# Guilucand/PanDelos

Measured on AMD Instinct MI355X. Metric: scored gene-pairs/sec (whole node), higher is better.
Workload: dtype u32 accumulate + f32 finalize

## Files before the change

pandelos_amd/csrc/pdl_api.hip:

```cpp
#include "pdl_common.h"

#include <algorithm>
#include <cstdlib>
#include <cstring>
#include <limits>

static thread_local std::string g_create_error = "";

#define PDL_GUARD_BEGIN try {
#define PDL_GUARD_END(ctx_)                                                       \
    } catch (const pdl_error &e) {                                                \
        if (ctx_) (ctx_)->err = e.msg; else g_create_error = e.msg;               \
        return e.code;                                                            \
    } catch (const std::bad_alloc &) {                                            \
        if (ctx_) (ctx_)->err = "host allocation failed";                         \
        return PDL_ERR_DEVICE;                                                    \
    }

template <class T> static T *xalloc(size_t n) {
    T *p = static_cast<T *>(malloc((n ? n : 1) * sizeof(T)));
    if (!p) throw std::bad_alloc();
    return p;
}

// ... 434 lines not shown
        ThreadCopier &tc = t_copier;
        tc.open(c->device);
        if (z) {
            tc.fetch(out->scores, c->c_score.as<float>() + z0, (size_t) z * 4);
            tc.fetch(out->percs, c->c_perc.as<float>() + z0, (size_t) z * 4);
            tc.fetch(out->tr_percs, c->c_tr.as<float>() + z0, (size_t) z * 4);
            tc.fetch(out->row, c->c_row.as<int32_t>() + z0, (size_t) z * 4);
            tc.fetch(out->column, c->c_col.as<int32_t>() + z0, (size_t) z * 4);
        }
        if (rows) tc.fetch(out->max_genome_score, c->MS.as<float>() + (size_t) p0 * G, (size_t) rows * G * 4);
        tc.fetch(out->max_genome_score_col, c->CM.as<float>() + (size_t) lg * N, (size_t) N * 4);
    }
    for (uint32_t i = 0; i < z; i++) {
        out->first_seq_genome[i] = (int32_t) c->h_genome_of[out->row[i]];
        out->second_seq_genome[i] = (int32_t) c->h_genome_of[out->column[i]];
    }
    for (uint32_t i = 0; i < N; i++) out->scoresMaxMappings[i] = std::numeric_limits<int32_t>::max();
    for (uint32_t j = 0; j < rows; j++) out->scoresMaxMappings[c->h_genome_rows[c->h_genome_row_off[genome] + j]] = (int32_t) j;
    return PDL_OK;
    } catch (const pdl_error &e) { { std::lock_guard<std::mutex> lk(c->mu); c->err = e.msg; } pdl_free_scores(out); return e.code;
    } catch (const std::bad_alloc &) { { std::lock_guard<std::mutex> lk(c->mu); c->err = "host allocation failed"; } pdl_free_scores(out); return PDL_ERR_DEVICE; }
}

void pdl_free_edges(pdl_edges *e) {
    if (!e) return;
    free(e->src); free(e->dst); free(e->score);
    memset(e, 0, sizeof(*e));
}

int pdl_compute_edges(pdl_ctx *c, uint32_t genome, pdl_edges *out) {
    if (!c || !out) return PDL_ERR_ARGUMENT;
    memset(out, 0, sizeof(*out));
    try {
    {
        std::lock_guard<std::mutex> lk(c->mu);
        int rc = c->scored ? PDL_OK : score_all_locked(c);
        if (rc != PDL_OK) return rc;
        if (genome >= c->G) PDL_FAIL(PDL_ERR_ARGUMENT, "genome %u out of range (%u genomes)", genome, c->G);
        if (c->h_local_genome[genome] < 0) PDL_FAIL(PDL_ERR_ARGUMENT, "genome %u is not in this context's shard", genome);
        if (!c->edges_valid) {
            PDL_HIP(hipSetDevice(c->device));
            pdl_run_bbh_all(c);
        }
    }
    const int32_t lg = c->h_local_genome[genome];
    const uint64_t a1 = c->h_edge1[lg], b1 = c->h_edge1[lg + 1], a2 = c->h_edge_off[lg], b2 = c->h_edge_off[lg + 1];
    const uint64_t n1 = c->n_edges1, n2 = c->n_edges - c->n_edges1;
    const uint32_t cnt = (uint32_t) ((b1 - a1) + (b2 - a2));
    out->count = cnt;
    out->src = xalloc<int32_t>(cnt); out->dst = xalloc<int32_t>(cnt); out->score = xalloc<float>(cnt);
    const uint8_t *m = c->edge_mirror;
    const size_t k1 = (size_t) (b1 - a1), k2 = (size_t) (b2 - a2);
    if (k1) {
        memcpy(out->src, m + a1 * 4, k1 * 4); memcpy(out->dst, m + n1 * 4 + a1 * 4, k1 * 4); memcpy(out->score, m + n1 * 8 + a1 * 4, k1 * 4);
    }
    if (k2) {
        const uint8_t *m2 = m + n1 * 12;
        memcpy(out->src + k1, m2 + a2 * 4, k2 * 4); memcpy(out->dst + k1, m2 + n2 * 4 + a2 * 4, k2 * 4); memcpy(out->score + k1, m2 + n2 * 8 + a2 * 4, k2 * 4);
    }
    return PDL_OK;
    } catch (const pdl_error &e) { { std::lock_guard<std::mutex> lk(c->mu); c->err = e.msg; } pdl_free_edges(out); return e.code;
    } catch (const std::bad_alloc &) { { std::lock_guard<std::mutex> lk(c->mu); c->err = "host allocation failed"; } pdl_free_edges(out); return PDL_ERR_DEVICE; }
}

void pdl_free_families(pdl_families *f) {
    if (!f) return;
    free(f->component_of); free(f->is_node); free(f->family_off); free(f->family_genes); free(f->collides);
    memset(f, 0, sizeof(*f));
}

static void fill_families(const pdl_fam_result &r, pdl_families *out) {
    out->sequences = r.sequences; out->nodes = r.nodes; out->families = r.families; out->colliding = r.colliding; out->device_ms = r.device_ms;
    out->component_of = xalloc<uint32_t>(r.component_of.size()); out->is_node = xalloc<uint8_t>(r.is_node.size());
    out->family_off = xalloc<uint32_t>(r.family_off.size()); out->family_genes = xalloc<uint32_t>(r.family_genes.size());
    out->collides = xalloc<uint8_t>(r.collides.size());
    if (!r.component_of.empty()) memcpy(out->component_of, r.component_of.data(), r.component_of.size() * 4);
    if (!r.is_node.empty()) memcpy(out->is_node, r.is_node.data(), r.is_node.size());
    memcpy(out->family_off, r.family_off.data(), r.family_off.size() * 4);
    if (!r.family_genes.empty()) memcpy(out->family_genes, r.family_genes.data(), r.family_genes.size() * 4);
    if (!r.collides.empty()) memcpy(out->collides, r.collides.data(), r.collides.size());
}

int pdl_compute_families(pdl_ctx *c, pdl_families *out) {
    if (!c || !out) return PDL_ERR_ARGUMENT;
    memset(out, 0, sizeof(*out));
    std::lock_guard<std::mutex> lk(c->mu);
    try {
        if (!c->preprocessed) PDL_FAIL(PDL_ERR_STATE, "pdl_compute_families before pdl_preprocess");
        if (c->only_complexity) PDL_FAIL(PDL_ERR_STATE, "pdl_compute_families: the context was preprocessed with only_complexity");
        if (c->dist) PDL_FAIL(PDL_ERR_STATE, "pdl_compute_families: not available on a multi-GPU context (gather the edges: pdl_families_of_edges)");
        if (c->shard_set || !c->dict_shard.empty())
            PDL_FAIL(PDL_ERR_STATE, "pdl_compute_families: a genome shard is in force, the context does not hold every genome's edges (gather them: pdl_families_of_edges)");
        int rc = c->scored ? PDL_OK : score_all_locked(c);
        if (rc != PDL_OK) return rc;
        PDL_HIP(hipSetDevice(c->device));
        if (!c->edges_valid) pdl_run_bbh_all(c);
        if (!c->fam_valid) pdl_run_families_of_context(c);
        fill_families(c->fam, out);
        return PDL_OK;
    } catch (const pdl_error &e) { c->err = e.msg; c->fam_valid = false; pdl_free_families(out); return e.code;
    } catch (const std::bad_alloc &) { c->err = "host allocation failed"; pdl_free_families(out); return PDL_ERR_DEVICE; }
}

int pdl_families_of_edges(pdl_ctx *c, const int32_t *src, const int32_t *dst, uint64_t n_edges, const uint32_t *genome_of, uint32_t n_sequences,
                          pdl_families *out) {
    if (!c || !out) return PDL_ERR_ARGUMENT;
    memset(out, 0, sizeof(*out));
    std::lock_guard<std::mutex> lk(c->mu);
    try {
        if ((n_edges && (!src || !dst)) || (n_sequences && !genome_of)) PDL_FAIL(PDL_ERR_ARGUMENT, "pdl_families_of_edges: NULL pointer");
        if (n_edges >= 0x7fffffffull || n_sequences >= 0x7fffffffu) PDL_FAIL(PDL_ERR_UNSUPPORTED, "pdl_families_of_edges: 2^31 genes or edges and more");
        PDL_HIP(hipSetDevice(c->device));
        pdl_ctx::FamBufs &b = c->fb;
        uint32_t g_max = 0;
        for (uint32_t i = 0; i < n_sequences; i++) g_max = std::max(g_max, genome_of[i]);
        if (n_edges) {
            b.up_src.alloc(n_edges * 4); b.up_dst.alloc(n_edges * 4);
            PDL_HIP(hipMemcpyAsync(b.up_src.p, src, n_edges * 4, hipMemcpyHostToDevice, c->stream));
            PDL_HIP(hipMemcpyAsync(b.up_dst.p, dst, n_edges * 4, hipMemcpyHostToDevice, c->stream));
        }
        if (n_sequences) {
            b.up_gen.alloc((size_t) n_sequences * 4);
            PDL_HIP(hipMemcpyAsync(b.up_gen.p, genome_of, (size_t) n_sequences * 4, hipMemcpyHostToDevice, c->stream));
        }
        const int32_t *s2[2] = {b.up_src.as<int32_t>(), nullptr}, *d2[2] = {b.up_dst.as<int32_t>(), nullptr};
        const uint64_t n2[2] = {n_edges, 0};
        pdl_fam_result r;
        pdl_run_families(c, s2, d2, n2, false, true, true, b.up_gen.as<uint32_t>(), n_sequences, bit_length64(g_max), r);
        fill_families(r, out);
        return PDL_OK;
    } catch (const pdl_error &e) { c->err = e.msg; pdl_free_families(out); return e.code;
    } catch (const std::bad_alloc &) { c->err = "host allocation failed"; pdl_free_families(out); return PDL_ERR_DEVICE; }
}

int pdl_set_option(pdl_ctx *c, const char *name, int64_t value) {
    if (!c || !name) return PDL_ERR_ARGUMENT;
    std::lock_guard<std::mutex> lk(c->mu);
    const std::string n(name);
    if (n == "join_tier1") {
        if (!(value == -1 || value == 0 || (value >= 9 && value <= 11) || value == 20 || value == 21)) { c->err = "join_tier1: -1, 0, 9, 10, 11, 20 or 21"; return PDL_ERR_ARGUMENT; }
        c->opt_tier1 = (int) value;
    } else if (n == "join_tier0") c->opt_tier0 = value < 0 ? -1 : (value != 0);
    else if (n == "sift_threshold") {
        if (value != 0 && value != 1) { c->err = "sift_threshold: 0 or 1"; return PDL_ERR_ARGUMENT; }
        c->opt_sift_threshold = (int) value;
    }
    else if (n == "join_tiny_tier2") c->opt_tiny_tier2 = value != 0;
    else if (n == "join_grid_pct") c->opt_grid_pct = (int) value;
    else if (n == "stage_timers") c->opt_stage_timers = value != 0;
    else if (n == "host_mirror") c->opt_host_mirror = value != 0;
    else if (n == "staging_cap") c->opt_staging_cap = value > 0 ? (uint64_t) value : 0;
    else if (n == "aside_test_reload") c->opt_aside_test_reload = value != 0;
    else if (n == "onepass_scan") c->opt_onepass_scan = value != 0;
    else if (n == "low_memory") c->opt_low_memory = value != 0;
    else if (n == "query_batch_bytes") {
        if (value <= 0) { c->err = "query_batch_bytes: a positive byte count"; return PDL_ERR_ARGUMENT; }
        c->opt_query_batch_bytes = (uint64_t) value;
        return PDL_OK;
    }
    else { c->err = "unknown option " + n; return PDL_ERR_ARGUMENT; }
    c->scored = false;
    return PDL_OK;
}

int pdl_dist_preprocess_begin(pdl_ctx *c, const uint8_t *d_residues, const uint64_t *d_offsets, const uint32_t *d_genome_of,
                              uint32_t n, uint64_t n_res, int k, uint32_t world, uint32_t rank, pdl_dist_slice *out) {
    if (!c || !out) return PDL_ERR_ARGUMENT;
    std::lock_guard<std::mutex> lk(c->mu);
    PDL_GUARD_BEGIN
    if (!d_offsets || !d_genome_of || (!d_residues && n_res)) PDL_FAIL(PDL_ERR_ARGUMENT, "null input pointer");
    if (((uintptr_t) d_residues & 15) != 0) PDL_FAIL(PDL_ERR_ARGUMENT, "d_residues must be 16-byte aligned");
    if (world == 0 || rank >= world || world > 64) PDL_FAIL(PDL_ERR_ARGUMENT, "rank %u of %u (at most 64 ranks)", rank, world);
    PDL_HIP(hipSetDevice(c->device));
    c->preprocessed = false; c->scored = false; c->tasks_ready = false; c->mirror_valid = false;
    c->dist = false; c->dist_stage = 0;
    adopt_device_input(c, d_residues, d_offsets, d_genome_of, n, n_res);
    c->N = n; c->R = n_res;
    c->U = c->Ushared = c->NG = c->P = c->M = 0;
    if (k <= 0) PDL_FAIL(PDL_ERR_KVALUE, "K value must be greater than 0.");
    if (n == 0) PDL_FAIL(PDL_ERR_EMPTY, "empty dataset");
    build_genome_layout(c);
    c->world = world; c->rank = rank;
    c->shard.clear(); c->shard_set = false; c->dict_shard.clear();
    pdl_run_dist_begin(c, k);
    out->d_postings = c->post.p; out->records = c->U_slice; out->kmers = c->M_slice;
    out->genome_weights = c->h_run_weights.data(); out->genomes = c->G;
    out->genome_costs = c->h_run_costs.data();
    return PDL_OK;
    PDL_GUARD_END(c)
}

int pdl_dist_preprocess_finish(pdl_ctx *c, void *d_postings_all, uint64_t total_records, const uint64_t *genome_weights, pdl_cost *out_cost) {
    if (!c) return PDL_ERR_ARGUMENT;
    std::lock_guard<std::mutex> lk(c->mu);
    PDL_GUARD_BEGIN
    if (!c->dist || c->dist_stage != 1) PDL_FAIL(PDL_ERR_STATE, "pdl_dist_preprocess_finish without pdl_dist_preprocess_begin");
    if (c->dist_sender) PDL_FAIL(PDL_ERR_STATE, "pdl_dist_preprocess_ranges built this run's range tuples (and took its group-head bits out): finish with pdl_dist_preprocess_finish_ranges");
    if (!d_postings_all || ((uintptr_t) d_postings_all & 7) != 0) PDL_FAIL(PDL_ERR_ARGUMENT, "the gathered dictionary must be an 8-byte aligned device array");
    if (total_records < c->U_slice) PDL_FAIL(PDL_ERR_ARGUMENT, "the gathered dictionary (%llu records) is smaller than this rank's run (%llu)",
                                             (unsigned long long) total_records, (unsigned long long) c->U_slice);
    PDL_HIP(hipSetDevice(c->device));
    c->post_ext = static_cast<uint2 *>(d_postings_all);
    pdl_run_dist_finish(c, total_records, genome_weights);
    c->preprocessed = true;
    fill_cost(c, out_cost);
    return PDL_OK;
    PDL_GUARD_END(c)
}

int pdl_dist_preprocess_ranges(pdl_ctx *c, const uint64_t *run_records, const uint64_t *genome_weights, const uint64_t *genome_costs, pdl_dist_ranges *out) {
    if (!c || !out || !run_records || !genome_weights || !genome_costs) return PDL_ERR_ARGUMENT;
    std::lock_guard<std::mutex> lk(c->mu);
    PDL_GUARD_BEGIN
    if (!c->dist || c->dist_stage != 1) PDL_FAIL(PDL_ERR_STATE, "pdl_dist_preprocess_ranges without pdl_dist_preprocess_begin");
    PDL_HIP(hipSetDevice(c->device));
    memset(out, 0, sizeof(*out));
    out->available = pdl_run_dist_ranges(c, run_records, genome_weights, genome_costs) ? 1 : 0;
    out->d_keys = c->dist_out_keys; out->d_ranges = reinterpret_cast<const uint64_t *>(c->dist_out_ranges);
    out->counts = c->h_tuple_counts.data(); out->total = c->dist_out_total;
    out->shared_records = c->dist_run_counters[0]; out->groups = c->dist_run_counters[1]; out->repeat_sample = c->dist_run_counters[2];
    return PDL_OK;
    PDL_GUARD_END(c)
}

int pdl_dist_preprocess_finish_ranges(pdl_ctx *c, void *d_postings_all, uint64_t total_records, uint32_t *d_keys, uint64_t *d_ranges, uint64_t n_tuples,
                                      const uint64_t *counter_sums, pdl_cost *out_cost) {
    if (!c || !counter_sums || ((!d_keys || !d_ranges) && n_tuples)) return PDL_ERR_ARGUMENT;
    std::lock_guard<std::mutex> lk(c->mu);
    PDL_GUARD_BEGIN
    if (!c->dist || c->dist_stage != 1 || !c->dist_sender) PDL_FAIL(PDL_ERR_STATE, "pdl_dist_preprocess_finish_ranges without a pdl_dist_preprocess_ranges that said \"available\"");
    if (!d_postings_all || ((uintptr_t) d_postings_all & 7) != 0) PDL_FAIL(PDL_ERR_ARGUMENT, "the gathered dictionary must be an 8-byte aligned device array");
    if (n_tuples && ((((uintptr_t) d_keys) & 3) != 0 || (((uintptr_t) d_ranges) & 7) != 0)) PDL_FAIL(PDL_ERR_ARGUMENT, "the received tuples must be aligned device arrays");
    PDL_HIP(hipSetDevice(c->device));
    c->post_ext = static_cast<uint2 *>(d_postings_all);
    pdl_run_dist_finish_ranges(c, total_records, d_keys, reinterpret_cast<unsigned long long *>(d_ranges), n_tuples, counter_sums);
    c->preprocessed = true;
    fill_cost(c, out_cost);
    return PDL_OK;
    PDL_GUARD_END(c)
}

int pdl_dist_genome_owner(const pdl_ctx *c, uint32_t *out) {
    if (!c || !out) return PDL_ERR_ARGUMENT;
    if (!c->dist || c->dist_stage < 2) return PDL_ERR_STATE;
    memcpy(out, c->h_owner.data(), (size_t) c->G * 4);
    return PDL_OK;
}

int pdl_dist_score_begin(pdl_ctx *c, pdl_dist_outbox *out) {
    if (!c || !out) return PDL_ERR_ARGUMENT;
    std::lock_guard<std::mutex> lk(c->mu);
    PDL_GUARD_BEGIN
    if (!c->dist || c->dist_stage < 2) PDL_FAIL(PDL_ERR_STATE, "pdl_dist_score_begin before pdl_dist_preprocess_finish");
    PDL_HIP(hipSetDevice(c->device));
    c->scored = false; c->mirror_valid = false; c->edges_valid = false; c->dist_stage = 2;
    pdl_run_dist_score_begin(c);
    out->d_cells = c->outbox.as<pdl_dist_cell>();
    out->counts = c->h_outbox_counts.data();
    out->total = 0;
    for (uint64_t v : c->h_outbox_counts) out->total += v;
    return PDL_OK;
    PDL_GUARD_END(c)
}

int pdl_dist_score_finish(pdl_ctx *c, const pdl_dist_cell *d_inbox, uint64_t n_inbox) {
    if (!c || (!d_inbox && n_inbox)) return PDL_ERR_ARGUMENT;
    std::lock_guard<std::mutex> lk(c->mu);
    PDL_GUARD_BEGIN
    if (!c->dist || c->dist_stage != 3) PDL_FAIL(PDL_ERR_STATE, "pdl_dist_score_finish without pdl_dist_score_begin");
    if (n_inbox >= 0xffffffffull) PDL_FAIL(PDL_ERR_UNSUPPORTED, "more than 2^32 received cells");
    PDL_HIP(hipSetDevice(c->device));
    pdl_run_dist_score_finish(c, d_inbox, n_inbox);
    return PDL_OK;
    PDL_GUARD_END(c)
}

int pdl_copy_device(pdl_ctx *c, void *d_dst, const void *d_src, uint64_t bytes) {
    if (!c || ((!d_dst || !d_src) && bytes)) return PDL_ERR_ARGUMENT;
    std::lock_guard<std::mutex> lk(c->mu);
    PDL_GUARD_BEGIN
    PDL_HIP(hipSetDevice(c->device));
    if (bytes) PDL_HIP(hipMemcpyAsync(d_dst, d_src, bytes, hipMemcpyDeviceToDevice, c->stream));
    PDL_HIP(hipStreamSynchronize(c->stream));
    return PDL_OK;
    PDL_GUARD_END(c)
}

int pdl_get_dictionary(pdl_ctx *c, uint64_t *ranks, uint32_t *seqs, uint32_t *counts) {
    if (!c) return PDL_ERR_ARGUMENT;
    std::lock_guard<std::mutex> lk(c->mu);
    PDL_GUARD_BEGIN
    if (!c->preprocessed) PDL_FAIL(PDL_ERR_STATE, "pdl_get_dictionary before pdl_preprocess");
    if (c->dist) PDL_FAIL(PDL_ERR_STATE, "pdl_get_dictionary: a multi-GPU context keeps ranks only for its own interval");
    if (!c->keys_b.p || !c->recpos.p) PDL_FAIL(PDL_ERR_STATE, "pdl_get_dictionary: the sorted k-mer stream was released (option low_memory)");
    PDL_HIP(hipSetDevice(c->device));
    const uint64_t U = c->U, M = c->M;
    std::vector<uint32_t> recpos(U);
    std::vector<uint2> post(U);
    PDL_HIP(hipMemcpyAsync(recpos.data(), c->recpos.p, U * 4, hipMemcpyDeviceToHost, c->stream));
    PDL_HIP(hipMemcpyAsync(post.data(), c->post.p, U * 8, hipMemcpyDeviceToHost, c->stream));
    std::vector<uint8_t> keys(M * (c->key64 ? 8 : 4));
    PDL_HIP(hipMemcpyAsync(keys.data(), c->keys_b.p, keys.size(), hipMemcpyDeviceToHost, c->stream));
    PDL_HIP(hipStreamSynchronize(c->stream));
    for (uint64_t u = 0; u < U; u++) {
        if (ranks) ranks[u] = c->key64 ? reinterpret_cast<uint64_t *>(keys.data())[recpos[u]]
                                       : (uint64_t) reinterpret_cast<uint32_t *>(keys.data())[recpos[u]];
// ... 154 lines not shown
```

pandelos_amd/csrc/pdl_common.h:

```cpp
#pragma once

#include <atomic>
#include <chrono>

#include <hip/hip_runtime.h>

#include <cstdint>
#include <cstdio>
#include <mutex>
#include <cstdlib>
#include <string>
#include <utility>
#include <vector>

#include "../../include/pandelos_amd.h"

#define PDL_WAVE 64

#ifdef __HIPCC__
__device__ __forceinline__ void pdl_sync() {
#ifndef PDL_PLAIN_SYNCTHREADS
    asm volatile("s_waitcnt lgkmcnt(0)" ::: "memory");
#endif
    __syncthreads();
// ... 59 lines not shown
    PDL_JC_CURSOR_T0 = 11,
    PDL_JC_ROWS_T0B = 12,
    PDL_JC_CURSOR_T0B = 13,
    PDL_JC_ROWS_T1 = 14,
    PDL_JC_WORDS = 16,
};
enum : uint32_t {
    PDL_JT_CTR_WORDS = 8,
    PDL_JT_EMITTED = 8,
    PDL_JT_RELOADS = PDL_JC_RELOADS,
    PDL_JT_ROWS_T1 = 11,
    PDL_JT_WORDS = 12,
};
static_assert(PDL_JC_ROWS_T1 < PDL_JC_WORDS && PDL_JC_RELOADS < PDL_JT_WORDS && PDL_JC_CURSOR_T3 + 1 == PDL_JT_CTR_WORDS, "join counter layout");

struct pdl_error {
    int code;
    std::string msg;
};

#define PDL_HIP(expr)                                                                           \
    do {                                                                                        \
        hipError_t _e = (expr);                                                                 \
        if (_e != hipSuccess) {                                                                 \
            throw pdl_error{PDL_ERR_DEVICE, std::string(#expr) + ": " + hipGetErrorString(_e)}; \
        }                                                                                       \
    } while (0)

#define PDL_FAIL(code_, ...)                                  \
    do {                                                      \
        char _b[512];                                         \
        snprintf(_b, sizeof(_b), __VA_ARGS__);                \
        throw pdl_error{(code_), std::string(_b)};            \
    } while (0)

struct DevBuf {
    void *p = nullptr;
    size_t bytes = 0;
    void alloc(size_t n) {
        if (n <= bytes && p) return;
        release();
        size_t want = n ? n : 16;
        PDL_HIP(hipMalloc(&p, want));
        bytes = want;
    }
    void release() {
        if (p) (void) hipFree(p);
        p = nullptr;
        bytes = 0;
    }
    template <class T> T *as() const { return static_cast<T *>(p); }
    ~DevBuf() { release(); }
    void grow_keep(size_t n, hipStream_t st) {
        if (n <= bytes && p) return;
        void *q = nullptr;
        PDL_HIP(hipMalloc(&q, n));
        if (p && bytes) {
            PDL_HIP(hipMemcpyAsync(q, p, bytes, hipMemcpyDeviceToDevice, st));
            PDL_HIP(hipStreamSynchronize(st));
            (void) hipFree(p);
        }
        p = q;
        bytes = n;
    }
    DevBuf() = default;
    DevBuf(const DevBuf &) = delete;
    DevBuf &operator=(const DevBuf &) = delete;
};

struct DevView {
    void *p = nullptr;
    template <class T> T *as() const { return static_cast<T *>(p); }
};

struct RankParams {
    uint8_t rank_values[256];
    uint64_t last_multiplier;
    uint32_t base;
    uint32_t k;
    uint32_t rank_bits;
    uint32_t hash_fallback;
    uint32_t key_bits;
};

struct EventPair {
    hipEvent_t a = nullptr, b = nullptr;
    bool used = false;
};

struct pdl_fam_result {
    uint32_t sequences = 0, nodes = 0, families = 0, colliding = 0;
    std::vector<uint32_t> component_of, family_off, family_genes;
    std::vector<uint8_t> is_node, collides;
    float device_ms = 0.f;
};

struct pdl_ctx {
    int device = 0;
    hipStream_t stream = nullptr;
    bool own_stream = false;
    uint32_t flags = 0;
    std::string err;
    std::mutex mu;

    const uint8_t *d_res = nullptr;
    const uint64_t *d_off = nullptr;
    const uint32_t *d_gen = nullptr;
    DevBuf in_res, in_off, in_gen;
    DevBuf own_gen;

    uint32_t *gen_pin = nullptr; size_t gen_pin_words = 0;
    hipEvent_t ev_gen = nullptr;
    bool layout_deferred = false;

    bool preprocessed = false;
    bool only_complexity = false;
    uint32_t N = 0, G = 0;
    uint64_t R = 0, M = 0, U = 0, Ushared = 0, NG = 0, P = 0, sum_kseq = 0, max_kseq = 0, min_kseq = 0;
    uint64_t Urepeat = 0;
    RankParams rp{};

    DevBuf ing_res, ing_off, ing_gen;
    uint8_t *ing_pin[2] = {nullptr, nullptr};
    size_t ing_pin_bytes = 0;
    hipEvent_t ing_ev[2] = {nullptr, nullptr};
    hipStream_t ing_stream = nullptr;
    std::vector<uint64_t> ing_h_off;
    std::vector<uint32_t> ing_h_gen;
    std::vector<std::string> ing_genome_names;
    uint64_t ing_R = 0;
    bool ingested = false;

    DevBuf kseq_len;
    DevBuf gene_len;
    DevBuf kmer_off;
    DevBuf cost;
    std::vector<uint64_t> h_genome_cost;

    DevBuf keys_a, keys_b, vals_a, vals_b, sort_tmp;
    bool key64 = false;
    DevBuf recpos;
    DevBuf post;
    DevBuf ranges;
    const uint2 *ranges8 = nullptr;
    DevBuf head_bits;
    bool costs_ready = true;
    DevBuf seq_off;
    bool upper_only = false;
    DevBuf scan_tmp;
    DevBuf lb_tile, lb_chunk, lb_ctr;
    uint32_t lb_epoch = 0;
    bool opt_low_memory = false;
    bool reshard_pending = false;
    bool opt_onepass_scan = false;
    DevBuf scratch;
    DevBuf scalars;

    std::vector<uint32_t> h_genome_of;
    std::vector<uint32_t> h_genome_row_off;
    std::vector<uint32_t> h_genome_rows;
    std::vector<uint32_t> shard;
    bool shard_set = false;
    std::vector<uint32_t> dict_shard;
    DevBuf seq_in_shard;
    DevBuf own_iv;
    std::vector<uint2> h_own_iv;
    std::vector<uint8_t> h_seq_in_shard;

    bool scored = false;
    uint32_t n_task_rows = 0;
    std::vector<int32_t> h_local_genome;
    std::vector<uint32_t> h_task_row_off;
    std::vector<uint64_t> h_cell_off;
    DevBuf task_blob;
    uint32_t *task_pin = nullptr; size_t task_pin_words = 0;
    hipStream_t copy_stream = nullptr; hipEvent_t ev_tasks = nullptr, ev_entry = nullptr;
    DevView task_rows;
    DevView task_lg;
    DevBuf row_desc;
    DevBuf MS;
    DevBuf CM;
    DevBuf row_base, row_cnt, fin_off;
    DevBuf st_score, st_perc, st_tr, st_col, st_first;
    uint64_t st_cap = 0;
    DevBuf c_score, c_perc, c_tr, c_row, c_col;
    uint64_t Z = 0;
    DevBuf join_ctr;
    DevBuf overflow_rows;
    DevBuf gene_info;
    DevBuf join_defer;
    DevBuf glb_table;
    bool glb_clean = false;
    DevBuf row_desc2;
    DevBuf mirror_cnt, mirror_ref;
    DevView taskpos_of;
    std::vector<uint32_t> h_fin;
    bool tasks_ready = false;
    DevBuf scratch2;
    DevBuf task_off;
    int cus = 0;
    uint32_t occ_tier1[5] = {0, 0, 0, 0, 0};
    uint32_t occ_tier0[2] = {0, 0}, occ_tier0b[2] = {0, 0};

    bool edges_valid = false;
    DevBuf bbh_kind, bbh_tab, e_src, e_dst, e_score;
    uint8_t *edge_mirror = nullptr;
    size_t edge_mirror_bytes = 0;
    uint64_t n_edges = 0, n_edges1 = 0;
    std::vector<uint32_t> h_bbh_at;
    std::vector<uint64_t> h_edge1, h_edge_off;

    int opt_tier1 = -1;
    int opt_tier0 = -1;
    int opt_sift_threshold = 1;
    bool opt_tiny_tier2 = false;
    bool opt_stage_timers = true;
    int opt_grid_pct = 0;
    bool opt_host_mirror = true;
    uint64_t opt_staging_cap = 0;
    bool opt_aside_test_reload = false;

    bool dist = false;
    uint32_t world = 1, rank = 0;
    int dist_stage = 0;
    uint2 *post_ext = nullptr;
    uint64_t U_slice = 0, M_slice = 0;
    std::vector<uint32_t> h_owner;
    std::vector<uint64_t> h_upper_cost;
    std::vector<uint64_t> h_run_weights;
    std::vector<uint64_t> h_run_costs;
    bool dist_sender = false;
    int dist_tail = -1;
    uint64_t run_base = 0, dist_total = 0;
    DevBuf seq_owner;
    DevBuf tuple_off;
    std::vector<uint64_t> h_tuple_counts;
    uint32_t *dist_out_keys = nullptr;
    unsigned long long *dist_out_ranges = nullptr;
    uint64_t dist_out_total = 0, dist_run_counters[3] = {0, 0, 0};
    DevBuf owner_of_genome;
    DevView local_genome;
    DevBuf outbox;
    DevBuf outbox_tab;
    std::vector<uint64_t> h_outbox_counts;
    uint64_t st_local = 0;
    uint64_t n_inbox = 0;
    uint32_t order_grid1 = 0;

    struct QueryBufs {
        DevBuf res, off, koff, kseq, keys_a, keys_b, vals_a, vals_b, recpos, post, desc, gkey, rec_sorted, row_lookups, row_off,
               fold, ctl, MS, CM, row_base, row_cnt, fin_off, rowid, overflow, st, cells, hbm;
        bool hbm_clean = false;
        uint32_t hbm_cols = 0, hbm_slots = 0;
        const uint32_t *rec_sorted_at = nullptr;
        hipEvent_t ev[6] = {};
        void release() {
            DevBuf *all[] = {&res, &off, &koff, &kseq, &keys_a, &keys_b, &vals_a, &vals_b, &recpos, &post, &desc, &gkey, &rec_sorted,
                             &row_lookups, &row_off, &fold, &ctl, &MS, &CM, &row_base, &row_cnt, &fin_off, &rowid, &overflow, &st, &cells, &hbm};
            for (DevBuf *b : all) b->release();
            hbm_clean = false; hbm_cols = hbm_slots = 0; rec_sorted_at = nullptr;
        }
    } qb;
    struct QueryBatchBufs {
        DevBuf res, off, koff, kseq, gene_begin, res_begin, gene_query, keys_a, keys_b, vals_a, vals_b, recpos, post, qkey, perm, srank, spost,
               seg_off, folds, desc, gkey, rec_sorted, row_lookups, row_off, ctl, MS, CM, row_base, row_cnt, fin_off, rowid, overflow, st, cells;
        hipEvent_t ev[6] = {};
        uint8_t *stage = nullptr; size_t stage_bytes = 0;
        void release() {
            if (stage) { (void) hipHostFree(stage); stage = nullptr; stage_bytes = 0; }
            DevBuf *all[] = {&res, &off, &koff, &kseq, &gene_begin, &res_begin, &gene_query, &keys_a, &keys_b, &vals_a, &vals_b, &recpos, &post, &qkey,
                             &perm, &srank, &spost, &seg_off, &folds, &desc, &gkey, &rec_sorted, &row_lookups, &row_off, &ctl, &MS, &CM, &row_base,
                             &row_cnt, &fin_off, &rowid, &overflow, &st, &cells};
            for (DevBuf *b : all) b->release();
        }
    } qbb;
    uint64_t opt_query_batch_bytes = 1ull << 30;
    struct FamBufs {
        DevBuf parent, comp, same_deg, is_node, collides, fam_off, fam_of_label, run_off, run_of;
        DevBuf mk_a, mk_b, mv_a, mv_b;
        DevBuf ck_a, ck_b, cv_a, cv_b;
        DevBuf ek_a, ek_b, ev_a, ev_b;
        DevBuf up_src, up_dst, up_gen;
        hipEvent_t ev[4] = {};
    } fb;
    bool fam_valid = false;
    pdl_fam_result fam;
    hipEvent_t app_ev[4] = {};
    struct RemoveBufs {
        DevBuf gmap;
        DevBuf gen_in;
        DevBuf new_id;
        DevBuf kseq, gen, glen;
        DevBuf tile;
        DevBuf ctl;
        hipEvent_t ev[4] = {};
    } rm;
    uint8_t alpha_present[256] = {};

    pdl_timings tm{};
    EventPair ev[16];
    uint8_t *pin = nullptr;
    uint8_t *pin_dev = nullptr;
    size_t pin_bytes = 0;
    uint32_t pin_epoch = 0;
    uint8_t *mirror = nullptr;
    size_t mirror_bytes = 0;
// ... 167 lines not shown
```

pandelos_amd/csrc/pdl_dict.hip:

```cpp
#include "pdl_common.h"
#include "pdl_scan.h"
#include "pdl_sort.h"
#include "pdl_append.h"
#include "pdl_remove.h"

#include <algorithm>
#include <cstring>

#define RABIN_MODULO 18446744073709551557ULL


__global__ __launch_bounds__(256) void k_zero_u64(uint64_t *p, size_t n) {
    for (size_t i = (size_t) blockIdx.x * 256 + threadIdx.x; i < n; i += (size_t) gridDim.x * 256) p[i] = 0;
}
constexpr int HIST_THREADS = 256;
__global__ __launch_bounds__(HIST_THREADS) void k_hist(const uint8_t *__restrict__ res, uint64_t n, unsigned long long *__restrict__ hist) {
    __shared__ uint32_t s_seen[256];
    s_seen[threadIdx.x] = 0;
    pdl_sync();
    const uint64_t n16 = n / 16;
    const uint4 *res16 = reinterpret_cast<const uint4 *>(res);
    const uint64_t stride = (uint64_t) gridDim.x * HIST_THREADS;
    auto mark = [&](const uint4 &v) {
        const uint32_t w[4] = {v.x, v.y, v.z, v.w};
#pragma unroll
        for (int j = 0; j < 4; j++) {
            s_seen[w[j] & 0xff] = 1u; s_seen[(w[j] >> 8) & 0xff] = 1u; s_seen[(w[j] >> 16) & 0xff] = 1u; s_seen[w[j] >> 24] = 1u;
        }
    };
    uint64_t i = (uint64_t) blockIdx.x * HIST_THREADS + threadIdx.x;
    for (; i + 3 * stride < n16; i += 4 * stride) {
        const uint4 v0 = res16[i], v1 = res16[i + stride], v2 = res16[i + 2 * stride], v3 = res16[i + 3 * stride];
        mark(v0); mark(v1); mark(v2); mark(v3);
    }
    for (; i < n16; i += stride) mark(res16[i]);
    if (blockIdx.x == 0)
        for (uint64_t t = n16 * 16 + threadIdx.x; t < n; t += HIST_THREADS) s_seen[res[t]] = 1u;
    pdl_sync();
    if (s_seen[threadIdx.x]) hist[threadIdx.x] = 1ull;
}

static void rank_init_host(RankParams &rp, const uint64_t counters[256], int kvalue) {
    memset(&rp, 0, sizeof(rp));
    rp.k = (uint32_t) kvalue;
    int rank = 0;
    for (int i = 0; i < 256; i++)
        if (counters[i] > 0) rp.rank_values[i] = (uint8_t) rank++;
    const uint8_t rank_base = (uint8_t) rank;
    rp.base = rank_base;
    uint64_t last_multiplier = 1;
    bool has_overflow = false;
    int tmp_kvalue = kvalue - 1;
    while (tmp_kvalue--) {
        uint64_t ovflw_test = last_multiplier;
        last_multiplier *= rank_base;
        if (has_overflow) {
            last_multiplier %= RABIN_MODULO;
        } else if ((ovflw_test > last_multiplier) || (ovflw_test * rank_base > last_multiplier * rank_base)) {
            has_overflow = true;
            last_multiplier = ((ovflw_test % RABIN_MODULO) * rank_base) % RABIN_MODULO;
        }
    }
    rp.last_multiplier = last_multiplier;
    rp.hash_fallback = has_overflow ? 1u : 0u;
    rp.key_bits = 64;
    if (has_overflow) {
        rp.rank_bits = 64;
    } else {
        uint64_t rank_tmp = last_multiplier * rank_base;
        rp.rank_bits = rank_tmp ? bit_length64(rank_tmp - 1) : 1;
        if (rp.rank_bits == 0) rp.rank_bits = 1;
        unsigned __int128 exact = 1;
        bool fits = true;
        for (int i = 0; i < kvalue && fits; i++) { exact *= rank_base; fits = (exact >> 64) == 0; }
        if (fits) rp.key_bits = rp.rank_bits;
    }
}

struct KseqFlag {
    const uint64_t *off; uint32_t k;
    __device__ uint32_t operator()(uint64_t i) const {
        const uint64_t b = off[i], e = off[i + 1];
        const uint64_t len = e >= b ? e - b : 0;
        return len >= k ? (uint32_t) (len - k + 1) : 0u;
    }
};
struct KseqApply {
    uint32_t *kseq_len; uint32_t *gene_len; uint64_t *kmer_off;
    unsigned long long *cost;
    const uint64_t *off; uint64_t n_res; unsigned long long *bad;
    __device__ void operator()(uint64_t i, uint32_t f, uint32_t prefix) const {
        kseq_len[i] = f;
        gene_len[i] = (uint32_t) (off[i + 1] - off[i]);
        kmer_off[i] = prefix;
        cost[i] = 0;
        if (off[i + 1] < off[i] || off[i + 1] > n_res) atomicOr(bad, 1ull);
    }
};

constexpr uint32_t RANK_SPAN = 128;
constexpr int RANK_THREADS = 256;
constexpr int RANK_ITEMS = 4;
constexpr int RANK_TILE = RANK_THREADS * RANK_ITEMS;

__device__ __forceinline__ uint32_t upper_bound_u64(const uint64_t *a, uint32_t lo, uint32_t hi, uint64_t v) {
    while (lo < hi) {
        uint32_t mid = lo + ((hi - lo) >> 1);
        if (a[mid] <= v) lo = mid + 1; else hi = mid;
    }
    return lo;
}

struct __attribute__((packed, aligned(1))) UnalignedU64 { uint64_t v; };
__device__ __forceinline__ uint64_t load_residues8(const uint8_t *__restrict__ res, uint64_t p, uint64_t n_res) {
    if (p + 8 <= n_res) return reinterpret_cast<const UnalignedU64 *>(res + p)->v;
    uint64_t w = 0;
    for (uint32_t b = 0; b < 8 && p + b < n_res; b++) w |= (uint64_t) res[p + b] << (8 * b);
    return w;
}

constexpr uint32_t DIST_BIN_BITS = 12, DIST_BINS = 1u << DIST_BIN_BITS;

template <class KeyT, int MODE>
__global__ __launch_bounds__(RANK_THREADS) void k_rank(const uint8_t *__restrict__ res, const uint64_t *__restrict__ off,
                                                       const uint64_t *__restrict__ kmer_off, uint32_t n_seq, uint64_t m, uint64_t n_res,
                                                       RankParams rp, KeyT *__restrict__ keys, uint32_t *__restrict__ vals,
                                                       uint32_t bin_shift, uint32_t *__restrict__ bins) {
    __shared__ uint8_t s_rv[256];
    __shared__ uint32_t s_lo, s_hi;
    __shared__ uint64_t s_koff[RANK_SPAN + 1], s_off[RANK_SPAN];
    __shared__ uint32_t s_bins[MODE == 1 ? DIST_BINS : 1];
    for (int i = threadIdx.x; i < 256; i += RANK_THREADS) s_rv[i] = rp.rank_values[i];
    if constexpr (MODE == 1) for (uint32_t i = threadIdx.x; i < DIST_BINS; i += RANK_THREADS) s_bins[i] = 0;
    const uint64_t tiles = (m + RANK_TILE - 1) / RANK_TILE;
  for (uint64_t tile = blockIdx.x; tile < tiles; tile += gridDim.x) {
    pdl_sync();
    const uint64_t q0 = tile * RANK_TILE;
    const uint64_t q_last = min(q0 + RANK_TILE, m) - 1;
    if (threadIdx.x == 0) s_lo = upper_bound_u64(kmer_off, 0, n_seq + 1, q0) - 1;
    if (threadIdx.x == 64) s_hi = upper_bound_u64(kmer_off, 0, n_seq + 1, q_last) - 1;
    pdl_sync();
    const uint32_t lo = s_lo, hi = s_hi;
    const uint32_t span = hi - lo + 1;
    const bool staged = span <= RANK_SPAN;
    if (staged) {
        for (uint32_t i = threadIdx.x; i <= span; i += RANK_THREADS) s_koff[i] = kmer_off[lo + i];
        for (uint32_t i = threadIdx.x; i < span; i += RANK_THREADS) s_off[i] = off[lo + i];
    }
    pdl_sync();
    const uint32_t k = rp.k;
    const KeyT base = (KeyT) rp.base;
    uint32_t sq[RANK_ITEMS];
    uint64_t pos[RANK_ITEMS];
#pragma unroll
    for (int j = 0; j < RANK_ITEMS; j++) {
        const uint64_t qj = q0 + (uint64_t) j * RANK_THREADS + threadIdx.x;
        const uint64_t q = qj < m ? qj : m - 1;
        if (staged) {
            uint32_t a = 0;
            if (span <= 8) {
#pragma unroll
                for (uint32_t i = 1; i < 8; i++) a += (uint32_t) (i < span && s_koff[i < span ? i : 0] <= q);
            } else {
                uint32_t b = span;
                while (a < b) { const uint32_t mid = (a + b) >> 1; if (s_koff[mid + 1] <= q) a = mid + 1; else b = mid; }
            }
            sq[j] = lo + a;
            pos[j] = s_off[a] + (q - s_koff[a]);
        } else {
            sq[j] = upper_bound_u64(kmer_off, lo, hi + 1, q) - 1;
            pos[j] = off[sq[j]] + (q - kmer_off[sq[j]]);
        }
    }
    KeyT r[RANK_ITEMS];
#pragma unroll
    for (int j = 0; j < RANK_ITEMS; j++) r[j] = 0;
    for (uint32_t c0 = 0; c0 < k; c0 += 8) {
        uint64_t w[RANK_ITEMS];
        bool safe = true;
#pragma unroll
        for (int j = 0; j < RANK_ITEMS; j++) safe = safe && pos[j] + c0 + 8 <= n_res;
        if (__all(safe)) {
#pragma unroll
            for (int j = 0; j < RANK_ITEMS; j++) w[j] = reinterpret_cast<const UnalignedU64 *>(res + pos[j] + c0)->v;
        } else {
#pragma unroll
            for (int j = 0; j < RANK_ITEMS; j++) w[j] = load_residues8(res, pos[j] + c0, n_res);
        }
        const uint32_t nb = min(8u, k - c0);
        for (uint32_t b = 0; b < nb; b++) {
#pragma unroll
            for (int j = 0; j < RANK_ITEMS; j++) r[j] = r[j] * base + s_rv[(uint32_t) (w[j] >> (8 * b)) & 0xffu];
        }
    }
#pragma unroll
    for (int j = 0; j < RANK_ITEMS; j++) {
        const uint64_t q = q0 + (uint64_t) j * RANK_THREADS + threadIdx.x;
        if (q < m) {
            if constexpr (MODE == 1) atomicAdd(&s_bins[(uint32_t) (r[j] >> bin_shift)], 1u);
            keys[q] = r[j]; vals[q] = sq[j];
        }
    }
  }
    if constexpr (MODE == 1) {
        pdl_sync();
        for (uint32_t i = threadIdx.x; i < DIST_BINS; i += RANK_THREADS) { const uint32_t v = s_bins[i]; if (v) atomicAdd(&bins[i], v); }
    }
}

__device__ __forceinline__ uint64_t update_rank_hash_dev(uint64_t current, uint64_t vnext, uint64_t vpop, uint64_t lm, uint64_t base) {
    uint64_t wrapped = current + RABIN_MODULO - vpop * lm;
    uint64_t lo = wrapped * base;
    uint64_t hi = __umul64hi(wrapped, base);
    uint64_t lo2 = lo + vnext;
    hi += (lo2 < lo);
    uint64_t t = hi * 59ull;
    uint64_t r = lo2 + t;
    if (r < lo2) r += 59ull;
    if (r >= RABIN_MODULO) r -= RABIN_MODULO;
    return r;
}

template <int MODE>
__global__ __launch_bounds__(256) void k_rank_hash(const uint8_t *__restrict__ res, const uint64_t *__restrict__ off,
                                                   const uint64_t *__restrict__ kmer_off, uint32_t n_seq, RankParams rp,
                                                   uint64_t *__restrict__ keys, uint32_t *__restrict__ vals, uint32_t *__restrict__ bins) {
    __shared__ uint8_t s_rv[256];
    for (int i = threadIdx.x; i < 256; i += 256) s_rv[i] = rp.rank_values[i];
    pdl_sync();
    const uint32_t s = blockIdx.x * 256 + threadIdx.x;
    if (s >= n_seq) return;
    const uint64_t b = off[s], e = off[s + 1];
    const uint32_t k = rp.k;
    if (e - b < k) return;
    const uint8_t *p = res + b;
    const uint64_t len = e - b;
    uint64_t q = kmer_off[s];
    uint64_t rank = 0;
    const uint64_t v0 = s_rv[0];
    for (uint32_t i = 0; i < k; i++) rank = update_rank_hash_dev(rank, s_rv[p[i]], v0, rp.last_multiplier, rp.base);
    if constexpr (MODE == 1) atomicAdd(&bins[rank >> (64 - DIST_BIN_BITS)], 1u);
    keys[q] = rank; vals[q] = s; q++;
    for (uint64_t i = k; i < len; i++) {
        rank = update_rank_hash_dev(rank, s_rv[p[i]], s_rv[p[i - k]], rp.last_multiplier, rp.base);
        if constexpr (MODE == 1) atomicAdd(&bins[rank >> (64 - DIST_BIN_BITS)], 1u);
        keys[q] = rank; vals[q] = s; q++;
    }
}

template <class KeyT> struct RecHead {
    const KeyT *keys; const uint32_t *vals;
    __device__ uint32_t operator()(uint64_t q) const {
        const uint64_t qp = q ? q - 1 : 0;
        const KeyT k0 = keys[q], k1 = keys[qp];
        const uint32_t v0 = vals[q], v1 = vals[qp];
        return (uint32_t) (q == 0) | (uint32_t) (k0 != k1) | (uint32_t) (v0 != v1);
    }
};
template <class KeyT> struct RecScatter {
    const KeyT *keys; const uint32_t *vals; uint64_t m;
    uint32_t *recpos; uint2 *post;
    struct Loaded { uint32_t val, run; uint8_t head; };
    __device__ Loaded load(uint64_t q, uint32_t) const {
        const uint64_t qp = q ? q - 1 : 0, qn = q + 1 < m ? q + 1 : q;
        const KeyT key = keys[q], kprev = keys[qp], knext = keys[qn];
        const uint32_t val = vals[q], vnext = vals[qn];
        const bool head = q == 0 || kprev != key;
        uint64_t j = q + 1;
        if (j < m && knext == key && vnext == val) {
            j++;
            while (j < m && keys[j] == key && vals[j] == val) j++;
        }
        return Loaded{val, (uint32_t) (j - q), (uint8_t) (head ? 1 : 0)};
    }
    __device__ void store(uint64_t q, uint32_t f, uint32_t prefix, const Loaded &v) const {
        if (!f) return;
        recpos[prefix] = (uint32_t) q;
        post[prefix] = make_uint2(v.val, v.run | ((uint32_t) v.head << 31));
    }
};

template <class KeyT> struct SelFlag {
    const KeyT *keys; uint32_t shift, b_lo, b_hi;
    __device__ uint32_t operator()(uint64_t q) const { const uint32_t b = (uint32_t) (keys[q] >> shift); return (uint32_t) (b >= b_lo) & (uint32_t) (b < b_hi); }
};
template <class KeyT> struct SelApply {
    const KeyT *keys; const uint32_t *vals; KeyT *keys_out; uint32_t *vals_out;
    struct Loaded { KeyT key; uint32_t val; };
    __device__ Loaded load(uint64_t q, uint32_t f) const { return f ? Loaded{keys[q], vals[q]} : Loaded{0, 0u}; }
    __device__ void store(uint64_t, uint32_t f, uint32_t prefix, const Loaded &v) const { if (f) { keys_out[prefix] = v.key; vals_out[prefix] = v.val; } }
};

constexpr uint32_t HEAD_BIT = 0x80000000u;
constexpr uint32_t GT_NONE = 0xffffffffu;
constexpr uint32_t COST_LDS_GENOMES = 4096;

__device__ __forceinline__ uint32_t find_head_back(const uint2 *post, uint32_t pos, uint32_t lane) {
    for (;;) {
        const uint32_t base = pos + 1 >= PDL_WAVE ? pos + 1 - PDL_WAVE : 0;
        const uint32_t idx = base + lane;
        const bool f = idx <= pos && ((post[idx <= pos ? idx : pos].y >> 31) || idx == 0);
        const unsigned long long m = __ballot(f);
        if (m) return base + 63u - (uint32_t) __clzll((long long) m);
        pos = base - 1;
    }
}
__device__ __forceinline__ uint32_t find_head_fwd(const uint2 *post, uint32_t pos, uint32_t n, uint32_t lane) {
    for (uint32_t base = pos; base < n; base += PDL_WAVE) {
        const uint32_t idx = base + lane;
        const bool f = idx < n && (post[idx < n ? idx : n - 1].y >> 31);
        const unsigned long long m = __ballot(f);
        if (m) return base + (uint32_t) __ffsll((long long) m) - 1u;
    }
    return n;
}

__global__ __launch_bounds__(1024) void k_fold_last_record(uint2 *__restrict__ post, uint32_t *__restrict__ recpos, const uint64_t *d_u) {
    __shared__ uint32_t s_gs, s_p;
    const uint32_t u_count = (uint32_t) *d_u;
    if (u_count < 2) return;
    const uint32_t lastp = u_count - 1;
    uint2 last = post[lastp];
    if (!(last.y >> 31)) return;
    last.y &= ~HEAD_BIT;
    const uint32_t last_rp = recpos ? recpos[lastp] : 0u;
    if (threadIdx.x < PDL_WAVE) {
        const uint32_t gs = find_head_back(post, lastp - 1, threadIdx.x);
        if (threadIdx.x == 0) {
            uint32_t lo = gs, hi = lastp;
            while (lo < hi) {
                const uint32_t mid = lo + ((hi - lo) >> 1);
                if (post[mid].x <= last.x) lo = mid + 1; else hi = mid;
            }
            s_gs = gs; s_p = lo;
        }
    }
    pdl_sync();
    const uint32_t p = s_p, gs = s_gs;
    if (p == lastp) { if (threadIdx.x == 0) post[lastp] = last; return; }
    for (uint32_t hi = lastp; hi > p; hi = hi > 1024 ? hi - 1024 : 0) {
        const bool live = hi >= 1 + threadIdx.x && hi - 1 - threadIdx.x >= p;
        const uint32_t i = hi - 1 - threadIdx.x;
        uint2 v = make_uint2(0, 0);
        uint32_t rp = 0;
        if (live) { v = post[i]; if (recpos) rp = recpos[i]; }
        pdl_sync();
        if (live) { post[i + 1] = v; if (recpos) recpos[i + 1] = rp; }
        pdl_sync();
        if (hi <= 1024) break;
    }
    if (threadIdx.x == 0) {
        if (p == gs) { last.y |= HEAD_BIT; post[gs + 1].y &= ~HEAD_BIT; }
        post[p] = last;
        if (recpos) recpos[p] = last_rp;
    }
}

struct GroupTileArgs {
    uint2 *post;
// ... 212 lines not shown
        gs = m ? ww * 64u + 63u - (uint32_t) __clzll((long long) m) : 0u;
    }
    {
        unsigned long long m = b == 63 ? 0ull : head_bits[w] & ~((2ull << b) - 1ull);
        uint32_t ww = w;
        while (!m && ww + 1 < words) m = head_bits[++ww];
        ge = m ? ww * 64u + (uint32_t) __ffsll((long long) m) - 1u : n;
        if (ge > n) ge = n;
    }
    if (ge - gs >= 2) atomicAdd(&cost[post[u].x], (unsigned long long) (ge - gs));
}

template <int MODE>
__global__ __launch_bounds__(GW_THREADS) void k_range_count(GroupTileArgs a) {
    extern __shared__ unsigned long long s_dyn[];
    __shared__ uint32_t s_red[2];
    uint2 *s_iv = reinterpret_cast<uint2 *>(s_dyn);
    const uint32_t n_iv = (MODE == 0 || MODE == 2) ? a.n_own_iv : 0u;
    if constexpr (MODE == 0 || MODE == 2) { for (uint32_t i = threadIdx.x; i < n_iv; i += GW_THREADS) s_iv[i] = a.own_iv[i]; }
    if (threadIdx.x < 2) s_red[threadIdx.x] = 0;
    pdl_sync();
    const uint32_t tid = threadIdx.x, lane = tid & (PDL_WAVE - 1);
    const uint32_t gw = blockIdx.x * GW_WAVES + tid / PDL_WAVE;
    const uint32_t n = (uint32_t) scan_count(a.n_bound, a.d_n);
    const uint32_t tiles = (n + GW_TILE - 1) / GW_TILE;
    uint32_t n_rec = 0, n_grp = 0, n_rep = 0;
    for (uint32_t tile = gw; tile < tiles; tile += gridDim.x * GW_WAVES) {
        const uint32_t t0 = tile * GW_TILE;
        uint2 po[GW_ROUNDS];
        uint32_t ynext[GW_ROUNDS];
#pragma unroll
        for (int j = 0; j < GW_ROUNDS; j++) {
            const uint32_t u = t0 + j * PDL_WAVE + lane;
            po[j] = a.post[u < n ? u : n - 1];
            ynext[j] = a.post[u + 1 < n ? u + 1 : n - 1].y;
        }
        uint32_t ins = 0xffffffffu;
        if constexpr (MODE == 0 || MODE == 2) {
            ins = 0;
            if (n_iv) {
                uint32_t lo_i[GW_ROUNDS], hi_i[GW_ROUNDS];
#pragma unroll
                for (int j = 0; j < GW_ROUNDS; j++) { lo_i[j] = 0; hi_i[j] = n_iv; }
                for (uint32_t span = n_iv; span > 0; span >>= 1) {
#pragma unroll
                    for (int j = 0; j < GW_ROUNDS; j++) {
                        const uint32_t mid = (lo_i[j] + hi_i[j]) >> 1;
                        const bool go = lo_i[j] < hi_i[j] && s_iv[mid < n_iv ? mid : n_iv - 1].x <= po[j].x;
                        if (lo_i[j] < hi_i[j]) { if (go) lo_i[j] = mid + 1; else hi_i[j] = mid; }
                    }
                }
#pragma unroll
                for (int j = 0; j < GW_ROUNDS; j++) ins |= (uint32_t) (lo_i[j] > 0 && po[j].x < s_iv[lo_i[j] > 0 ? lo_i[j] - 1 : 0].y) << j;
            } else {
                uint8_t inb[GW_ROUNDS];
#pragma unroll
                for (int j = 0; j < GW_ROUNDS; j++) inb[j] = a.in_shard[po[j].x];
#pragma unroll
                for (int j = 0; j < GW_ROUNDS; j++) ins |= (uint32_t) (inb[j] != 0) << j;
            }
        }
        uint32_t cnt = 0, first_h = GT_NONE, last_h = 0, any_h = 0;
#pragma unroll
        for (int j = 0; j < GW_ROUNDS; j++) {
            const uint32_t u = t0 + j * PDL_WAVE + lane;
            const bool live = u < n;
            const bool head = live && (po[j].y >> 31);
            const bool next_head = u + 1 >= n || (ynext[j] >> 31);
            const bool shared = live && !(head && next_head);
            bool r = MODE == 0 ? shared : (live && !next_head);
            if constexpr (MODE == 0 || MODE == 2) r = r && ((ins >> j) & 1u);
            cnt += r;
            n_rec += shared; n_grp += head && !next_head;
            if (head) { first_h = min(first_h, u); last_h = max(last_h, u); any_h = 1; }
        }
        if ((tile & 7u) == 0) {
#pragma unroll
            for (int j = 0; j < GW_ROUNDS; j++) n_rep += 8u * (uint32_t) (t0 + j * PDL_WAVE + lane < n && (po[j].y & ~HEAD_BIT) >= 2u);
        }
#pragma unroll
        for (int d = PDL_WAVE / 2; d > 0; d >>= 1) {
            cnt += __shfl_xor(cnt, d, PDL_WAVE);
            first_h = min(first_h, (uint32_t) __shfl_xor((int) first_h, d, PDL_WAVE));
            last_h = max(last_h, (uint32_t) __shfl_xor((int) last_h, d, PDL_WAVE));
            any_h |= (uint32_t) __shfl_xor((int) any_h, d, PDL_WAVE);
        }
        if (lane == 0) { a.tile_sums[tile] = cnt; a.th_first[tile] = first_h; a.th_last[tile] = any_h ? last_h : GT_NONE; }
    }
#pragma unroll
    for (int d = PDL_WAVE / 2; d > 0; d >>= 1) { n_rec += __shfl_xor(n_rec, d, PDL_WAVE); n_grp += __shfl_xor(n_grp, d, PDL_WAVE); n_rep += __shfl_xor(n_rep, d, PDL_WAVE); }
    if (lane == 0) { atomicAdd(&s_red[0], n_rec); atomicAdd(&s_red[1], n_grp); if (n_rep) atomicAdd(&a.counters[3], (unsigned long long) n_rep); }
    pdl_sync();
    if (tid < 2 && s_red[tid]) atomicAdd(&a.counters[tid], (unsigned long long) s_red[tid]);
}

static_assert(GW_WAVES * GW_TILE == (int) PDL_RADIX_TILE && GW_THREADS == (int) PDL_RADIX_BINS, "a workgroup's four tiles are one tile of the radix pass");
__global__ __launch_bounds__(GW_THREADS) void k_range_count_hist(GroupTileArgs a, uint32_t n_tiles4, uint32_t *__restrict__ counts) {
    __shared__ uint32_t s_h[PDL_RADIX_BINS];
    __shared__ uint32_t s_red[2];
    const uint32_t tid = threadIdx.x, lane = tid & (PDL_WAVE - 1), wave = tid / PDL_WAVE;
    const uint32_t n = (uint32_t) scan_count(a.n_bound, a.d_n);
    if (tid < 2) s_red[tid] = 0;
    uint32_t n_rec = 0, n_grp = 0, n_rep = 0;
    for (uint32_t blk = blockIdx.x; blk < n_tiles4; blk += gridDim.x) {
        s_h[tid] = 0;
        pdl_sync();
        const uint32_t tile = blk * GW_WAVES + wave, t0 = tile * GW_TILE;
        if (t0 < n) {
            uint2 po[GW_ROUNDS];
            uint32_t ynext[GW_ROUNDS];
#pragma unroll
            for (int j = 0; j < GW_ROUNDS; j++) {
                const uint32_t u = t0 + j * PDL_WAVE + lane;
                po[j] = a.post[u < n ? u : n - 1];
                ynext[j] = a.post[u + 1 < n ? u + 1 : n - 1].y;
            }
            uint32_t cnt = 0, first_h = GT_NONE, last_h = 0, any_h = 0;
#pragma unroll
            for (int j = 0; j < GW_ROUNDS; j++) {
                const uint32_t u = t0 + j * PDL_WAVE + lane;
                const bool live = u < n;
                const bool head = live && (po[j].y >> 31);
                const bool next_head = u + 1 >= n || (ynext[j] >> 31);
                const bool r = live && !next_head;
                if (r) atomicAdd(&s_h[po[j].x & (PDL_RADIX_BINS - 1)], 1u);
                cnt += r;
                n_rec += live && !(head && next_head); n_grp += head && !next_head;
                if (head) { first_h = min(first_h, u); last_h = max(last_h, u); any_h = 1; }
            }
#pragma unroll
            for (int d = PDL_WAVE / 2; d > 0; d >>= 1) {
                cnt += __shfl_xor(cnt, d, PDL_WAVE);
                first_h = min(first_h, (uint32_t) __shfl_xor((int) first_h, d, PDL_WAVE));
                last_h = max(last_h, (uint32_t) __shfl_xor((int) last_h, d, PDL_WAVE));
                any_h |= (uint32_t) __shfl_xor((int) any_h, d, PDL_WAVE);
            }
            if (lane == 0) { a.tile_sums[tile] = cnt; a.th_first[tile] = first_h; a.th_last[tile] = any_h ? last_h : GT_NONE; }
            if ((tile & 7u) == 0) {
#pragma unroll
                for (int j = 0; j < GW_ROUNDS; j++) n_rep += 8u * (uint32_t) (t0 + j * PDL_WAVE + lane < n && (po[j].y & ~HEAD_BIT) >= 2u);
            }
        }
        pdl_sync();
        counts[(size_t) tid * n_tiles4 + blk] = s_h[tid];
    }
#pragma unroll
    for (int d = PDL_WAVE / 2; d > 0; d >>= 1) { n_rec += __shfl_xor(n_rec, d, PDL_WAVE); n_grp += __shfl_xor(n_grp, d, PDL_WAVE); n_rep += __shfl_xor(n_rep, d, PDL_WAVE); }
    if (lane == 0) { atomicAdd(&s_red[0], n_rec); atomicAdd(&s_red[1], n_grp); if (n_rep) atomicAdd(&a.counters[3], (unsigned long long) n_rep); }
    pdl_sync();
    if (tid < 2 && s_red[tid]) atomicAdd(&a.counters[tid], (unsigned long long) s_red[tid]);
}

__global__ __launch_bounds__(GW_THREADS) void k_range_scatter(GroupTileArgs a, uint32_t n_tiles4, const uint32_t *__restrict__ offs,
                                                              uint32_t *__restrict__ keys_out, unsigned long long *__restrict__ vals_out) {
    const uint32_t n = (uint32_t) scan_count(a.n_bound, a.d_n);
    if ((uint64_t) blockIdx.x * PDL_RADIX_TILE >= n) return;
    __shared__ uint32_t s_key[PDL_RADIX_TILE];
    __shared__ unsigned long long s_val[PDL_RADIX_TILE];
    __shared__ uint16_t s_cnt[GW_WAVES][PDL_RADIX_BINS];
    __shared__ uint32_t s_tile_off[PDL_RADIX_BINS];
    __shared__ uint32_t s_goff[PDL_RADIX_BINS];
    __shared__ uint32_t s_wsum[17];
    __shared__ unsigned long long s_own;
    const uint32_t tid = threadIdx.x, lane = tid & (PDL_WAVE - 1), wave = tid / PDL_WAVE;
    const uint32_t tiles = (n + GW_TILE - 1) / GW_TILE;
    const uint32_t tile = blockIdx.x * GW_WAVES + wave, t0 = tile * GW_TILE, t1 = min(t0 + (uint32_t) GW_TILE, n);
    const bool active = tile < tiles;
    for (int w = 0; w < GW_WAVES; w++) s_cnt[w][tid] = 0;
    s_goff[tid] = offs[(size_t) tid * n_tiles4 + blockIdx.x];
    if (tid == 0) s_own = 0;
    pdl_sync();

    const unsigned long long lt_mask = (1ull << lane) - 1ull, le_mask = (2ull << lane) - 1ull;
    uint2 po[GW_ROUNDS];
    unsigned long long val[GW_ROUNDS];
    uint16_t rank[GW_ROUNDS];
    uint32_t rbits = 0;
    unsigned long long own_lookups = 0;
#pragma unroll
    for (int j = 0; j < GW_ROUNDS; j++) {
        const uint32_t u = t0 + j * PDL_WAVE + lane;
        po[j] = a.post[u < n ? u : n - 1];
    }
    if (active) {
        const uint32_t hb = lane < tile ? a.th_last[tile - 1 - lane] : GT_NONE;
        const uint32_t ha = tile + 1 + lane < tiles ? a.th_first[tile + 1 + lane] : GT_NONE;
        unsigned long long m[GW_ROUNDS];
#pragma unroll
        for (int j = 0; j < GW_ROUNDS; j++) m[j] = __ballot(t0 + j * PDL_WAVE + lane < n && (po[j].y >> 31));
        uint32_t before = t0;
        if (!(m[0] & 1ull)) {
            unsigned long long hm = __ballot(hb != GT_NONE);
            if (hm) before = (uint32_t) __shfl((int) hb, __ffsll((long long) hm) - 1, PDL_WAVE);
            else {
                before = 0;
                for (uint32_t hi = tile >= PDL_WAVE ? tile - PDL_WAVE : 0; hi > 0;) {
                    const uint32_t base = hi >= PDL_WAVE ? hi - PDL_WAVE : 0, idx = base + lane;
                    const uint32_t v = idx < hi ? a.th_last[idx] : GT_NONE;
                    hm = __ballot(v != GT_NONE);
                    if (hm) { before = (uint32_t) __shfl((int) v, 63 - __clzll((long long) hm), PDL_WAVE); break; }
                    hi = base;
                }
            }
        }
        uint32_t after;
        {
            unsigned long long hm = __ballot(ha != GT_NONE);
            if (hm) after = (uint32_t) __shfl((int) ha, __ffsll((long long) hm) - 1, PDL_WAVE);
            else {
                after = n;
                for (uint32_t lo = tile + 1 + PDL_WAVE; lo < tiles; lo += PDL_WAVE) {
                    const uint32_t idx = lo + lane;
                    const uint32_t v = idx < tiles ? a.th_first[idx] : GT_NONE;
                    hm = __ballot(v != GT_NONE);
                    if (hm) { after = (uint32_t) __shfl((int) v, __ffsll((long long) hm) - 1, PDL_WAVE); break; }
                }
            }
        }
        before = (uint32_t) __builtin_amdgcn_readfirstlane((int) before);
        after = (uint32_t) __builtin_amdgcn_readfirstlane((int) after);
        uint32_t nextr[GW_ROUNDS];
        uint32_t nx = after;
#pragma unroll
        for (int j = GW_ROUNDS - 1; j >= 0; j--) {
            nextr[j] = nx;
            if (m[j]) nx = t0 + j * PDL_WAVE + (uint32_t) __ffsll((long long) m[j]) - 1u;
        }
        uint32_t pr = before;
#pragma unroll
        for (int j = 0; j < GW_ROUNDS; j++) {
            const uint32_t u = t0 + j * PDL_WAVE + lane;
            const unsigned long long at_or_below = m[j] & le_mask, above = m[j] & ~le_mask;
            const uint32_t gs = at_or_below ? t0 + j * PDL_WAVE + 63u - (uint32_t) __clzll((long long) at_or_below) : pr;
            const uint32_t ge = above ? t0 + j * PDL_WAVE + (uint32_t) __ffsll((long long) above) - 1u : nextr[j];
            const bool live = u < t1;
            const bool shared = live && ge - gs >= 2;
            const bool r = shared && u + 1 < ge;
            const uint32_t cnt = po[j].y & ~HEAD_BIT;
            if (live && (po[j].y >> 31)) a.post[u].y = cnt;
            if (shared) own_lookups += ge - gs;
            val[j] = (unsigned long long) (u + 1) | ((unsigned long long) ((ge - u - 1) | (min(cnt, 1023u) << 22)) << 32);
            rbits |= (uint32_t) r << j;
            if (lane == 0) a.head_bits[(size_t) tile * GW_ROUNDS + j] = m[j];
            if (m[j]) pr = t0 + j * PDL_WAVE + 63u - (uint32_t) __clzll((long long) m[j]);
        }
    }
#pragma unroll
    for (int j = 0; j < GW_ROUNDS; j++) {
        const bool valid = (rbits >> j) & 1u;
        const uint32_t d = po[j].x & (PDL_RADIX_BINS - 1);
        unsigned long long same = __ballot(valid);
#pragma unroll
        for (int b = 0; b < 8; b++) {
            const unsigned long long mb = __ballot((d >> b) & 1u);
            same &= ((d >> b) & 1u) ? mb : ~mb;
        }
        const uint32_t seen = s_cnt[wave][d];
        rank[j] = (uint16_t) (seen + (uint32_t) __popcll(same & lt_mask));
        if (valid && (same & lt_mask) == 0) s_cnt[wave][d] = (uint16_t) (seen + (uint32_t) __popcll(same));
    }
    pdl_sync();
    uint32_t tot = 0;
    uint32_t wcnt[GW_WAVES];
#pragma unroll
    for (int w = 0; w < GW_WAVES; w++) { wcnt[w] = s_cnt[w][tid]; tot += wcnt[w]; }
    uint32_t tile_total;
    const uint32_t ex = block_exclusive_scan_u32(tot, s_wsum, tile_total);
    s_tile_off[tid] = ex;
    uint32_t run = ex;
#pragma unroll
    for (int w = 0; w < GW_WAVES; w++) { s_cnt[w][tid] = (uint16_t) run; run += wcnt[w]; }
    pdl_sync();
#pragma unroll
    for (int j = 0; j < GW_ROUNDS; j++) {
        if ((rbits >> j) & 1u) {
            const uint32_t lp = s_cnt[wave][po[j].x & (PDL_RADIX_BINS - 1)] + rank[j];
            s_key[lp] = po[j].x;
            s_val[lp] = val[j];
        }
    }
#pragma unroll
    for (int d = PDL_WAVE / 2; d > 0; d >>= 1) own_lookups += __shfl_xor(own_lookups, d, PDL_WAVE);
    if (lane == 0 && own_lookups) atomicAdd(&s_own, own_lookups);
    pdl_sync();
#pragma unroll
    for (int j = 0; j < GW_ROUNDS; j++) {
        const uint32_t e = j * GW_THREADS + tid;
        if (e < tile_total) {
            const uint32_t k = s_key[e];
            const uint32_t d = k & (PDL_RADIX_BINS - 1);
            const uint64_t dst = (uint64_t) s_goff[d] + (e - s_tile_off[d]);
            keys_out[dst] = k;
            vals_out[dst] = s_val[e];
        }
    }
    if (tid == 0 && s_own) atomicAdd(&a.counters[2], s_own);
}

__global__ __launch_bounds__(256) void k_tile_prefix(uint32_t *__restrict__ tile_sums, const uint64_t *d_n, uint64_t n_bound,
                                                     uint32_t *__restrict__ chunk_sums, uint32_t n_blocks) {
    const uint32_t b = blockIdx.x * 4 + threadIdx.x / PDL_WAVE, lane = threadIdx.x & (PDL_WAVE - 1);
    if (b >= n_blocks) return;
    const uint32_t tiles = (uint32_t) ((scan_count(n_bound, d_n) + GW_TILE - 1) / GW_TILE);
    const uint32_t t = b * PDL_WAVE + lane;
    const uint32_t v = t < tiles ? tile_sums[t] : 0u;
    const uint32_t inc = wave_inclusive_scan_u32(v);
    if (t < tiles) tile_sums[t] = inc - v;
    if (lane == PDL_WAVE - 1) chunk_sums[b] = inc;
}

__global__ __launch_bounds__(256) void k_genes_of_rank(const uint32_t *__restrict__ genome_of, const uint32_t *__restrict__ owner, uint32_t rank,
                                                       uint32_t n_seq, uint8_t *__restrict__ in_shard) {
    const uint32_t s = blockIdx.x * 256 + threadIdx.x;
    if (s < n_seq) in_shard[s] = owner[genome_of[s]] == rank ? 1 : 0;
}
__global__ __launch_bounds__(256) void k_gene_owner(const uint32_t *__restrict__ genome_of, const uint32_t *__restrict__ owner, uint32_t n_seq,
                                                    uint8_t *__restrict__ seq_owner) {
    const uint32_t s = blockIdx.x * 256 + threadIdx.x;
    if (s < n_seq) seq_owner[s] = (uint8_t) owner[genome_of[s]];
}
__global__ __launch_bounds__(256) void k_owner_keys(uint32_t *__restrict__ key, const uint64_t *d_n, const uint8_t *__restrict__ seq_owner) {
    const uint32_t n = (uint32_t) *d_n;
    for (uint32_t i = blockIdx.x * 256 + threadIdx.x; i < n; i += gridDim.x * 256) {
        const uint32_t g = key[i];
        key[i] = g | ((uint32_t) seq_owner[g] << 24);
    }
}

__global__ __launch_bounds__(256) void k_gather_ranges(const uint32_t *__restrict__ idx_sorted, const uint32_t *__restrict__ key_sorted,
                                                       const uint4 *__restrict__ tuples, const uint64_t *d_n, uint4 *__restrict__ ranges,
                                                       unsigned long long *__restrict__ cost) {
    const uint32_t n = (uint32_t) *d_n;
    const uint32_t e = blockIdx.x * 256 + threadIdx.x;
    if (blockIdx.x * 256u >= n) return;
    const uint32_t lane = threadIdx.x & (PDL_WAVE - 1);
    const bool live = e < n;
    uint32_t g = 0xffffffffu;
    unsigned long long w = 0;
    if (live) {
        const uint4 t = tuples[idx_sorted[e]];
        ranges[e] = t;
        g = key_sorted[e];
        w = t.w;
    }
    unsigned long long todo = __ballot(live);
    while (todo) {
        const int leader = __ffsll((long long) todo) - 1;
        const uint32_t gl = __shfl(g, leader, PDL_WAVE);
        const bool in = live && g == gl;
        unsigned long long sum = in ? w : 0ull;
#pragma unroll
        for (int d = PDL_WAVE / 2; d > 0; d >>= 1) sum += __shfl_xor(sum, d, PDL_WAVE);
        if ((int) lane == leader) atomicAdd(&cost[gl], sum);
        todo &= ~__ballot(in);
    }
}
__global__ __launch_bounds__(256) void k_seq_offsets(const uint32_t *__restrict__ key_sorted, const uint64_t *d_n, uint32_t n_seq,
                                                     uint32_t *__restrict__ seq_off, uint32_t shift = 0, uint32_t mask = 0xffffffffu) {
    const uint32_t n = (uint32_t) *d_n;
    const uint32_t s = blockIdx.x * 256 + threadIdx.x;
    if (s > n_seq) return;
    uint32_t lo = 0, hi = n;
    while (lo < hi) {
        uint32_t mid = lo + ((hi - lo) >> 1);
        if (((key_sorted[mid] >> shift) & mask) < s) lo = mid + 1; else hi = mid;
    }
    seq_off[s] = lo;
}

__global__ __launch_bounds__(256) void k_genome_cost(const unsigned long long *__restrict__ cost, const uint32_t *__restrict__ kseq_len,
                                                     const uint32_t *__restrict__ genome_of, uint32_t n_seq,
                                                     unsigned long long *__restrict__ genome_cost, unsigned long long *__restrict__ sum_kseq,
                                                     unsigned long long *__restrict__ max_kseq, unsigned long long *__restrict__ min_kseq) {
    __shared__ unsigned long long s_sum, s_max, s_min;
    if (threadIdx.x == 0) { s_sum = 0; s_max = 0; s_min = ~0ull; }
    pdl_sync();
    const uint32_t lane = threadIdx.x & (PDL_WAVE - 1);
    unsigned long long ksum = 0, kmax = 0, kmin = ~0ull;
    for (uint32_t s0 = blockIdx.x * 256; s0 < n_seq; s0 += gridDim.x * 256) {
        const uint32_t s = s0 + threadIdx.x;
        const bool live = s < n_seq;
        unsigned long long c = live ? cost[s] : 0ull;
        const unsigned long long kl = live ? (unsigned long long) kseq_len[s] : 0ull;
        const uint32_t g = live ? genome_of[s] : 0xffffffffu;
        ksum += kl; kmax = kl > kmax ? kl : kmax; if (kl && kl < kmin) kmin = kl;
        const uint32_t g0 = __shfl(g, 0, PDL_WAVE);
        if (__all(g == g0 || !live)) {
            unsigned long long csum = c;
#pragma unroll
            for (int d = PDL_WAVE / 2; d > 0; d >>= 1) csum += __shfl_down(csum, d, PDL_WAVE);
            if (lane == 0 && csum && g0 != 0xffffffffu) atomicAdd(&genome_cost[g0], csum);
        } else if (live && c) {
            atomicAdd(&genome_cost[g], c);
        }
    }
#pragma unroll
    for (int d = PDL_WAVE / 2; d > 0; d >>= 1) {
        ksum += __shfl_down(ksum, d, PDL_WAVE);
        unsigned long long o = __shfl_down(kmax, d, PDL_WAVE);
        kmax = o > kmax ? o : kmax;
        o = __shfl_down(kmin, d, PDL_WAVE);
        kmin = o < kmin ? o : kmin;
    }
    if (lane == 0) { atomicAdd(&s_sum, ksum); atomicMax(&s_max, kmax); atomicMin(&s_min, kmin); }
    pdl_sync();
    if (threadIdx.x == 0 && s_sum) { atomicAdd(sum_kseq, s_sum); atomicMax(max_kseq, s_max); atomicMax(min_kseq, ~s_min); }
}

static void launch_genome_cost(pdl_ctx *c, size_t w_sum, size_t w_max) {
    static_assert(PDL_CTL_KSEQ_NMIN == PDL_CTL_KSEQ_MAX + 1 && PDL_CTL_LAZY_KSEQ_MAX + 1 <= PDL_CTL_LAST, "~min sits behind max");
    unsigned long long *d_scal = c->scalars.as<unsigned long long>();
    hipLaunchKernelGGL(k_genome_cost, dim3(std::min<uint32_t>((c->N + 255) / 256, 128)), dim3(256), 0, c->stream, c->cost.as<unsigned long long>(),
                       c->kseq_len.as<uint32_t>(), c->d_gen, c->N, d_scal + PDL_CTL_GCOST, d_scal + w_sum, d_scal + w_max, d_scal + w_max + 1);
    PDL_HIP(hipGetLastError());
}


static void stage_alphabet_and_lengths(pdl_ctx *c, int kvalue, bool only_complexity) {
    hipStream_t st = c->stream;
    if (kvalue <= 0) PDL_FAIL(PDL_ERR_KVALUE, "K value must be greater than 0.");
    const size_t ctl_words = PDL_CTL_GCOST + 2 * (size_t) (c->layout_deferred ? c->N : c->G);
    c->scalars.alloc(ctl_words * sizeof(uint64_t));
    uint64_t *d_scal = c->scalars.as<uint64_t>();
    hipLaunchKernelGGL(k_zero_u64, dim3((uint32_t) std::min<size_t>((ctl_words + 255) / 256, 1024)), dim3(256), 0, st, d_scal, ctl_words);

    ev_begin(c, EV_HIST);
    c->kseq_len.alloc((size_t) c->N * sizeof(uint32_t));
    c->gene_len.alloc((size_t) c->N * sizeof(uint32_t));
    c->kmer_off.alloc(((size_t) c->N + 1) * sizeof(uint64_t));
    c->cost.alloc((size_t) c->N * sizeof(uint64_t));
    scan_and_apply(c, c->N, KseqFlag{c->d_off, (uint32_t) kvalue},
                   KseqApply{c->kseq_len.as<uint32_t>(), c->gene_len.as<uint32_t>(), c->kmer_off.as<uint64_t>(), c->cost.as<unsigned long long>(), c->d_off, c->R,
                             reinterpret_cast<unsigned long long *>(d_scal + PDL_CTL_BAD_OFFSETS)}, d_scal + PDL_CTL_KMERS, c->kmer_off.as<uint64_t>() + c->N);
    if (c->layout_deferred) pdl_input_arrived(c);
    if (c->R) {
        uint32_t blocks = (uint32_t) std::min<uint64_t>((c->R / 64 + HIST_THREADS - 1) / HIST_THREADS + 1, 2048);
        hipLaunchKernelGGL(k_hist, dim3(blocks), dim3(HIST_THREADS), 0, st, c->d_res, c->R,
                           reinterpret_cast<unsigned long long *>(d_scal + PDL_CTL_HIST));
    }
    uint64_t counters[256];
    uint64_t M = 0, bad = 0;
    {
        PinRead rd(c);
        const uint64_t *pc = rd.add<uint64_t>(d_scal, PDL_CTL_GCOST);
        ev_end(c, EV_HIST);
        rd.sync();
        memcpy(counters, pc + PDL_CTL_HIST, sizeof(counters));
        M = pc[PDL_CTL_KMERS]; bad = pc[PDL_CTL_BAD_OFFSETS];
    }
    if (bad) PDL_FAIL(PDL_ERR_ARGUMENT, "offsets must ascend from 0 to the residue count (%llu)", (unsigned long long) c->R);
    rank_init_host(c->rp, counters, kvalue);
    for (int i = 0; i < 256; i++) c->alpha_present[i] = counters[i] ? 1 : 0;
    c->M = M;
    c->only_complexity = only_complexity;
    if (M == 0) PDL_FAIL(PDL_ERR_EMPTY, "no gene is at least k=%d residues long: the dictionary is empty", kvalue);
    if (c->R >= 0xfffffff0ull) PDL_FAIL(PDL_ERR_UNSUPPORTED, "more than 2^32 residues (%llu) need 64-bit stream positions", (unsigned long long) c->R);
    c->key64 = c->rp.rank_bits > 32;
}

template <class KeyT>
static void stage_rank(pdl_ctx *c, uint32_t *d_bins = nullptr, uint32_t bin_shift = 0) {
    hipStream_t st = c->stream;
    const uint64_t M = c->M;
    c->keys_a.alloc(M * sizeof(KeyT)); c->keys_b.alloc(M * sizeof(KeyT));
    c->vals_a.alloc(M * sizeof(uint32_t)); c->vals_b.alloc(M * sizeof(uint32_t));
    if (c->rp.hash_fallback) {
        if constexpr (sizeof(KeyT) == 8) {
            if (d_bins) hipLaunchKernelGGL(k_rank_hash<1>, dim3((c->N + 255) / 256), dim3(256), 0, st, c->d_res, c->d_off,
                                           c->kmer_off.as<uint64_t>(), c->N, c->rp, c->keys_a.as<uint64_t>(), c->vals_a.as<uint32_t>(), d_bins);
            else hipLaunchKernelGGL(k_rank_hash<0>, dim3((c->N + 255) / 256), dim3(256), 0, st, c->d_res, c->d_off,
                                    c->kmer_off.as<uint64_t>(), c->N, c->rp, c->keys_a.as<uint64_t>(), c->vals_a.as<uint32_t>(), (uint32_t *) nullptr);
        }
    } else {
        const uint64_t tiles = (M + RANK_TILE - 1) / RANK_TILE;
        if (d_bins) hipLaunchKernelGGL((k_rank<KeyT, 1>), dim3((uint32_t) std::min<uint64_t>(tiles, 2048)), dim3(RANK_THREADS), 0, st, c->d_res, c->d_off,
                                       c->kmer_off.as<uint64_t>(), c->N, M, c->R, c->rp, c->keys_a.as<KeyT>(), c->vals_a.as<uint32_t>(), bin_shift, d_bins);
        else hipLaunchKernelGGL((k_rank<KeyT, 0>), dim3((uint32_t) tiles), dim3(RANK_THREADS), 0, st, c->d_res, c->d_off,
                                c->kmer_off.as<uint64_t>(), c->N, M, c->R, c->rp, c->keys_a.as<KeyT>(), c->vals_a.as<uint32_t>(), 0u, (uint32_t *) nullptr);
    }
    PDL_HIP(hipGetLastError());
}

template <class KeyT>
static void stage_dedup(pdl_ctx *c, uint64_t m) {
    uint64_t *d_scal = c->scalars.as<uint64_t>();
    const KeyT *skeys = c->keys_b.as<KeyT>();
    const uint32_t *svals = c->vals_b.as<uint32_t>();
    ev_begin(c, EV_DICT);
    c->recpos.alloc((m + 1) * sizeof(uint32_t));
    c->post.alloc(m * sizeof(uint2));
    scan_and_apply(c, m, RecHead<KeyT>{skeys, svals},
                   RecScatter<KeyT>{skeys, svals, m, c->recpos.as<uint32_t>(), c->post.as<uint2>()}, d_scal + PDL_CTL_RECORDS);
}

template <class KeyT>
static void stage_sort_and_dedup(pdl_ctx *c, KeyT *keys_in, KeyT *keys_out, uint32_t *vals_in, uint32_t *vals_out, uint64_t m) {
    ev_begin(c, EV_SORT1);
    pdl_sort_pairs<KeyT>(c, keys_in, keys_out, vals_in, vals_out, m, c->rp.rank_bits, false, nullptr, 0, c->rp.key_bits == c->rp.rank_bits);
    ev_end(c, EV_SORT1);
    if ((void *) keys_out != c->keys_b.p) { std::swap(c->keys_a.p, c->keys_b.p); std::swap(c->keys_a.bytes, c->keys_b.bytes); }
    if ((void *) vals_out != c->vals_b.p) { std::swap(c->vals_a.p, c->vals_b.p); std::swap(c->vals_a.bytes, c->vals_b.bytes); }
    stage_dedup<KeyT>(c, m);
}

static uint32_t group_tiles_plan(pdl_ctx *c, GroupTileArgs &a) {
    const uint64_t tiles = (a.n_bound + GW_TILE - 1) / GW_TILE;
    if (tiles > 0x7fffffffull) PDL_FAIL(PDL_ERR_UNSUPPORTED, "dictionary of %llu records exceeds the grid limit", (unsigned long long) a.n_bound);
    const int cus = pdl_cus(c);
    a.n_blocks = (uint32_t) ((tiles + PDL_WAVE - 1) / PDL_WAVE);
    const uint32_t grid = (uint32_t) std::max<uint64_t>(1, std::min<uint64_t>((tiles + GW_WAVES - 1) / GW_WAVES, (uint64_t) cus * 8));
    c->scan_tmp.alloc(((size_t) tiles * 3 + a.n_blocks + 1) * sizeof(uint32_t));
    a.tile_sums = c->scan_tmp.as<uint32_t>(); a.th_first = a.tile_sums + tiles; a.th_last = a.th_first + tiles; a.chunk_sums = a.th_last + tiles;
    return grid;
}
template <int PASS, int MODE, bool GENOMES, bool RECORD_COSTS>
static void launch_group_tiles(pdl_ctx *c, const GroupTileArgs &a, uint32_t grid) {
    size_t dyn = GENOMES && a.n_genomes <= COST_LDS_GENOMES ? 2 * (size_t) a.n_genomes * sizeof(uint64_t) : 0;
    if (MODE == 0 || MODE == 2) dyn = (size_t) a.n_own_iv * sizeof(uint2);
    hipLaunchKernelGGL((k_group_waves<PASS, MODE, GENOMES, RECORD_COSTS>), dim3(grid), dim3(GW_THREADS), dyn, c->stream, a);
    PDL_HIP(hipGetLastError());
}

static void stage_ranges_and_costs(pdl_ctx *c, uint64_t bound, int mode, bool only_complexity) {
    hipStream_t st = c->stream;
    c->costs_ready = true; c->ranges8 = nullptr;
    uint64_t *d_scal = c->scalars.as<uint64_t>();
    const uint64_t *d_u = d_scal + PDL_CTL_RECORDS;
    uint2 *post = pdl_postings(c);
    GroupTileArgs ga{};
    ga.post = post; ga.n_bound = bound; ga.d_n = d_u;
    const uint32_t grid = group_tiles_plan(c, ga);
    ga.cost = c->cost.as<unsigned long long>();
    ga.counters = reinterpret_cast<unsigned long long *>(d_scal + PDL_CTL_COUNTERS);
    ga.genome_of = c->d_gen; ga.n_genomes = c->G;
    hipLaunchKernelGGL(k_fold_last_record, dim3(1), dim3(1024), 0, st, post, c->post_ext ? (uint32_t *) nullptr : c->recpos.as<uint32_t>(), d_u);
    if (only_complexity) {
        launch_group_tiles<0, 3, false, true>(c, ga, grid);
    } else {
        ev_begin(c, EV_SORT2);
        const bool packed = mode != 0 && c->N < (1u << 22);
        const bool exact = mode != 1;
        uint64_t cap = bound;
        uint4 *tuples = nullptr;
        unsigned long long *pay_a = nullptr, *pay_b = nullptr;
        uint32_t *k2a = nullptr, *v2a = nullptr, *k2b = nullptr, *v2b = nullptr;
        auto carve = [&]() {
            c->scratch.alloc(cap * (packed ? 2 * sizeof(uint64_t) + sizeof(uint32_t) : sizeof(uint4) + 3 * sizeof(uint32_t)) + (exact ? cap * sizeof(uint32_t) : 0) + 64);
            tuples = c->scratch.as<uint4>();
            pay_a = c->scratch.as<unsigned long long>(); pay_b = pay_a + cap;
            v2a = packed ? nullptr : reinterpret_cast<uint32_t *>(tuples + cap);
            k2b = packed ? reinterpret_cast<uint32_t *>(pay_b + cap) : v2a + cap;
            v2b = packed ? nullptr : k2b + cap;
            if (exact) k2a = (packed ? k2b : v2b) + cap;
            else { c->vals_a.alloc(cap * sizeof(uint32_t)); k2a = c->vals_a.as<uint32_t>(); }
        };
        if (!exact) carve();
        if (mode != 1) {
            std::vector<uint2> &iv = c->h_own_iv;
            iv.clear();
            bool contiguous = true;
            for (uint32_t g : c->dict_shard) {
                const uint32_t b0 = c->h_genome_row_off[g], e0 = c->h_genome_row_off[g + 1];
                if (b0 == e0) continue;
                const uint32_t first = c->h_genome_rows[b0], last = c->h_genome_rows[e0 - 1];
                if (last - first + 1 != e0 - b0) { contiguous = false; break; }
                if (!iv.empty() && iv.back().y == first) iv.back().y = last + 1; else iv.push_back(make_uint2(first, last + 1));
            }
            if (contiguous) std::sort(iv.begin(), iv.end(), [](const uint2 &p, const uint2 &q) { return p.x < q.x; });
            for (size_t i = 1; contiguous && i < iv.size(); i++) if (iv[i].x < iv[i - 1].y) contiguous = false;
            if (contiguous && !iv.empty() && iv.size() <= GW_MAX_IV) {
                c->own_iv.alloc(iv.size() * sizeof(uint2));
                PDL_HIP(hipMemcpyAsync(c->own_iv.p, iv.data(), iv.size() * sizeof(uint2), hipMemcpyHostToDevice, st));
                ga.own_iv = c->own_iv.as<uint2>(); ga.n_own_iv = (uint32_t) iv.size();
            }
        }
        if (mode != 1 && c->dist) {
            ga.in_shard = c->seq_in_shard.as<uint8_t>();
        } else if (mode != 1) {
            std::vector<uint8_t> &h = c->h_seq_in_shard;
            h.assign((size_t) c->N, 0);
            std::vector<uint8_t> gsel((size_t) c->G, 0);
            for (uint32_t g : c->dict_shard) gsel[g] = 1;
            for (uint32_t i = 0; i < c->N; i++) h[i] = gsel[c->h_genome_of[i]];
            c->seq_in_shard.alloc(c->N);
            PDL_HIP(hipMemcpyAsync(c->seq_in_shard.p, h.data(), c->N, hipMemcpyHostToDevice, st));
            ga.in_shard = c->seq_in_shard.as<uint8_t>();
        }
        c->head_bits.alloc(((bound + GW_TILE - 1) / GW_TILE) * GW_ROUNDS * sizeof(uint64_t));
        ga.head_bits = c->head_bits.as<unsigned long long>();
        const uint64_t *d_us = d_scal + PDL_CTL_RANGES;
        const bool fused = mode == 1 && packed;
        if (fused) {
            const uint32_t n_tiles4 = (uint32_t) ((bound + PDL_RADIX_TILE - 1) / PDL_RADIX_TILE);
            const size_t table = (size_t) PDL_RADIX_BINS * n_tiles4, tiles = (bound + GW_TILE - 1) / GW_TILE;
            c->sort_tmp.alloc((2 * table + 3 * tiles + 1) * sizeof(uint32_t));
            uint32_t *counts = c->sort_tmp.as<uint32_t>(), *offs = counts + table;
            ga.tile_sums = offs + table; ga.th_first = ga.tile_sums + tiles; ga.th_last = ga.th_first + tiles; ga.chunk_sums = nullptr;
            const uint32_t grid4 = std::max<uint32_t>(1, std::min<uint32_t>(n_tiles4, (uint32_t) c->cus * 8));
            hipLaunchKernelGGL(k_range_count_hist, dim3(grid4), dim3(GW_THREADS), 0, st, ga, n_tiles4, counts);
            pdl_radix_offsets(c, counts, offs, n_tiles4, d_scal + PDL_CTL_RANGES);
            hipLaunchKernelGGL(k_range_scatter, dim3(n_tiles4), dim3(GW_THREADS), 0, st, ga, n_tiles4, offs, k2b, pay_b);
            PDL_HIP(hipGetLastError());
        } else {
        {
            const size_t dyn = (size_t) ga.n_own_iv * sizeof(uint2);
            if (mode == 1) hipLaunchKernelGGL(k_range_count<1>, dim3(grid), dim3(GW_THREADS), 0, st, ga);
            else if (mode == 2) hipLaunchKernelGGL(k_range_count<2>, dim3(grid), dim3(GW_THREADS), dyn, st, ga);
            else hipLaunchKernelGGL(k_range_count<0>, dim3(grid), dim3(GW_THREADS), dyn, st, ga);
            PDL_HIP(hipGetLastError());
        }
        hipLaunchKernelGGL(k_tile_prefix, dim3((ga.n_blocks + 3) / 4), dim3(256), 0, st, ga.tile_sums, ga.d_n, ga.n_bound, ga.chunk_sums, ga.n_blocks);
        hipLaunchKernelGGL(k_scan_tile_scan, dim3(1), dim3(1024), 0, st, ga.chunk_sums, ga.n_blocks, d_scal + PDL_CTL_RANGES, (uint64_t *) nullptr);
        if (exact) {
            if (!c->tasks_ready) pdl_prepare_tasks(c);
            PinRead rd(c);
            const uint64_t *pn = rd.add<uint64_t>(d_us, 1);
            rd.sync();
            cap = std::max<uint64_t>(pn[0], 1);
            carve();
        }
        ga.key2 = k2a; ga.tuples = tuples; ga.pay8 = packed ? pay_a : nullptr;
        if (mode == 1) launch_group_tiles<1, 1, false, false>(c, ga, grid);
        else if (mode == 2) launch_group_tiles<1, 2, false, false>(c, ga, grid);
        else launch_group_tiles<1, 0, false, false>(c, ga, grid);
        }
        c->upper_only = mode != 0;
        const uint32_t seq_bits = std::max<uint32_t>(1, bit_length64(c->N ? c->N - 1 : 0));
        uint64_t n_sort = bound;
        const uint64_t *d_sort_n = d_us;
        if (exact) { n_sort = cap; d_sort_n = nullptr; }
        c->seq_off.alloc(((size_t) c->N + 1) * sizeof(uint32_t));
        if (packed) {
            if (fused) {
                std::swap(k2a, k2b); std::swap(pay_a, pay_b);
                pdl_sort_pairs<uint32_t, unsigned long long>(c, k2a, k2b, pay_a, pay_b, n_sort, seq_bits, false, d_sort_n, 8, true);
            } else
            pdl_sort_pairs<uint32_t, unsigned long long>(c, k2a, k2b, pay_a, pay_b, n_sort, seq_bits, false, d_sort_n, 0, true);
            ev_end(c, EV_SORT2);
            ev_begin(c, EV_RANGES);
            c->ranges8 = reinterpret_cast<const uint2 *>(pay_b);
            c->costs_ready = false;
        } else {
            pdl_sort_pairs<uint32_t>(c, k2a, k2b, v2a, v2b, n_sort, seq_bits, true, d_sort_n, 0, true);
            ev_end(c, EV_SORT2);
            ev_begin(c, EV_RANGES);
            c->ranges8 = nullptr;
            c->ranges.alloc(std::max<uint64_t>(n_sort, 1) * sizeof(uint4));
            const uint32_t gblocks = (uint32_t) std::max<uint64_t>((n_sort + 255) / 256, 1);
            hipLaunchKernelGGL(k_gather_ranges, dim3(gblocks), dim3(256), 0, st, v2b, k2b, tuples, d_us, c->ranges.as<uint4>(), c->cost.as<unsigned long long>());
        }
        hipLaunchKernelGGL(k_seq_offsets, dim3((c->N + 1 + 255) / 256), dim3(256), 0, st, k2b, d_us, c->N, c->seq_off.as<uint32_t>());
        PDL_HIP(hipGetLastError());
        ev_end(c, EV_RANGES);
    }

    launch_genome_cost(c, PDL_CTL_KSEQ_SUM, PDL_CTL_KSEQ_MAX);

    uint64_t own_cost = 0;
    {
        PinRead rd(c);
        const uint64_t *pt = rd.add<uint64_t>(d_scal, PDL_CTL_GCOST + (size_t) c->G);
        const uint32_t *lbe = lookback_error_word(c, rd);
        rd.sync();
        lookback_check(c, lbe);
        c->h_genome_cost.assign(pt + PDL_CTL_GCOST, pt + PDL_CTL_GCOST + c->G);
        c->U = pt[PDL_CTL_RECORDS];
        c->Ushared = pt[PDL_CTL_SHARED];
        c->Urepeat = pt[PDL_CTL_REPEATS];
        c->NG = pt[PDL_CTL_GROUPS];
        c->sum_kseq = pt[PDL_CTL_KSEQ_SUM];
        c->max_kseq = pt[PDL_CTL_KSEQ_MAX];
        c->min_kseq = pt[PDL_CTL_KSEQ_NMIN] == 0 ? 1 : ~pt[PDL_CTL_KSEQ_NMIN];
        own_cost = pt[PDL_CTL_OWN_COST];
    }
    c->P = 0;
    if (c->costs_ready) for (uint64_t v : c->h_genome_cost) c->P += v;
    else c->P = own_cost;
}

__global__ __launch_bounds__(256) void k_restore_heads(uint2 *__restrict__ post, const unsigned long long *__restrict__ head_bits, uint32_t n) {
    const uint32_t u = blockIdx.x * 256 + threadIdx.x;
    if (u >= n) return;
    if ((head_bits[u >> 6] >> (u & 63u)) & 1ull) post[u].y |= HEAD_BIT;
}

void pdl_run_reshard(pdl_ctx *c) {
    hipStream_t st = c->stream;
    if (c->dist || c->post_ext) PDL_FAIL(PDL_ERR_STATE, "genome shard: a multi-GPU context deals the genomes itself");
    if (c->dict_shard.empty() || c->upper_only) PDL_FAIL(PDL_ERR_STATE, "genome shard: the dictionary was built for all genomes; set the first shard before pdl_preprocess");
    uint64_t *d_scal = c->scalars.as<uint64_t>();
    const uint32_t n = (uint32_t) c->U;
    ev_begin(c, EV_PRE_TOTAL);
    hipLaunchKernelGGL(k_restore_heads, dim3((n + 255) / 256), dim3(256), 0, st, c->post.as<uint2>(), c->head_bits.as<unsigned long long>(), n);
    PDL_HIP(hipMemsetAsync(d_scal + PDL_CTL_RANGES, 0, sizeof(uint64_t), st));
    PDL_HIP(hipMemsetAsync(d_scal + PDL_CTL_COUNTERS, 0, (PDL_CTL_LAST - PDL_CTL_COUNTERS + 1) * sizeof(uint64_t), st));
    PDL_HIP(hipMemsetAsync(d_scal + PDL_CTL_GCOST, 0, 2 * (size_t) c->G * sizeof(uint64_t), st));
    PDL_HIP(hipMemsetAsync(c->cost.p, 0, (size_t) c->N * sizeof(uint64_t), st));
    const uint64_t sum_kseq = c->sum_kseq, max_kseq = c->max_kseq, min_kseq = c->min_kseq;
    PDL_HIP(hipMemsetAsync(d_scal + PDL_CTL_KSEQ_SUM, 0, sizeof(uint64_t), st));
    PDL_HIP(hipMemsetAsync(d_scal + PDL_CTL_KSEQ_MAX, 0, (PDL_CTL_KSEQ_NMIN - PDL_CTL_KSEQ_MAX + 1) * sizeof(uint64_t), st));
    c->dict_shard = c->shard;
    c->tasks_ready = false;
    ev_begin(c, EV_DICT); ev_end(c, EV_DICT);
    stage_ranges_and_costs(c, c->U, 0, false);
    c->sum_kseq = sum_kseq; c->max_kseq = max_kseq; c->min_kseq = min_kseq;
    ev_end(c, EV_PRE_TOTAL);
    PDL_HIP(hipStreamSynchronize(st));
    c->tm.sort_seq_ms = ev_ms(c, EV_SORT2);
    c->tm.ranges_ms = ev_ms(c, EV_RANGES);
    c->tm.reshard_ms = ev_ms(c, EV_PRE_TOTAL);
}

void pdl_ensure_costs(pdl_ctx *c) {
    if (c->costs_ready) return;
    hipStream_t st = c->stream;
    uint64_t *d_scal = c->scalars.as<uint64_t>();
    PDL_HIP(hipMemsetAsync(c->cost.p, 0, (size_t) c->N * sizeof(uint64_t), st));
    PDL_HIP(hipMemsetAsync(d_scal + PDL_CTL_GCOST, 0, (size_t) c->G * sizeof(uint64_t), st));
    const uint32_t n = (uint32_t) c->U;
    hipLaunchKernelGGL(k_gene_costs_lazy, dim3((n + 255) / 256), dim3(256), 0, st, pdl_postings(c), c->head_bits.as<unsigned long long>(), n,
                       c->cost.as<unsigned long long>());
    launch_genome_cost(c, PDL_CTL_LAZY_KSEQ_SUM, PDL_CTL_LAZY_KSEQ_MAX);
    PinRead rd(c);
    const uint64_t *pg = rd.add<uint64_t>(d_scal + PDL_CTL_GCOST, c->G);
    rd.sync();
    c->h_genome_cost.assign(pg, pg + c->G);
    c->costs_ready = true;
}

template <class KeyT>
static void dictionary_pipeline(pdl_ctx *c, bool only_complexity) {
    const uint64_t M = c->M;
    ev_begin(c, EV_RANK);
    stage_rank<KeyT>(c);
    ev_end(c, EV_RANK);
    KeyT *keys_in = c->keys_a.as<KeyT>(), *keys_out = c->keys_b.as<KeyT>();
    uint32_t *vals_in = c->vals_a.as<uint32_t>(), *vals_out = c->vals_b.as<uint32_t>();
    stage_sort_and_dedup<KeyT>(c, keys_in, keys_out, vals_in, vals_out, M);
    ev_end(c, EV_DICT);
    if (c->layout_deferred) pdl_finish_layout(c);
    if (!only_complexity) pdl_prepare_tasks(c);
    stage_ranges_and_costs(c, M, c->dict_shard.empty() ? 1 : 0, only_complexity);
    if (c->opt_low_memory) {
        PDL_HIP(hipStreamSynchronize(c->stream));
        c->keys_a.release(); c->keys_b.release(); c->vals_a.release(); c->vals_b.release(); c->recpos.release(); c->sort_tmp.release();
        if (c->ranges8 == nullptr) {}
    }
}

template <class KeyT>
static void rank_new_genes(pdl_ctx *c, const uint8_t *res, const uint64_t *off, const uint64_t *kmer_off, uint32_t n, uint64_t m, uint64_t n_res,
                           KeyT *keys, uint32_t *vals) {
    hipStream_t st = c->stream;
    if (c->rp.hash_fallback) {
        if constexpr (sizeof(KeyT) == 8)
            hipLaunchKernelGGL(k_rank_hash<0>, dim3((n + 255) / 256), dim3(256), 0, st, res, off, kmer_off, n, c->rp, keys, vals, (uint32_t *) nullptr);
    } else {
        const uint64_t tiles = (m + RANK_TILE - 1) / RANK_TILE;
        hipLaunchKernelGGL((k_rank<KeyT, 0>), dim3((uint32_t) tiles), dim3(RANK_THREADS), 0, st, res, off, kmer_off, n, m, n_res, c->rp,
                           keys, vals, 0u, (uint32_t *) nullptr);
    }
    PDL_HIP(hipGetLastError());
}

template <class KeyT>
static const void *query_dictionary(pdl_ctx *c, const uint8_t *res, const uint64_t *off, const uint64_t *kmer_off, uint32_t n, uint64_t m,
                                    uint64_t n_res, KeyT *keys_in, KeyT *keys_out, uint32_t *vals_in, uint32_t *vals_out, uint32_t *recpos,
                                    uint2 *post, uint64_t *d_u) {
    rank_new_genes<KeyT>(c, res, off, kmer_off, n, m, n_res, keys_in, vals_in);
    pdl_sort_pairs<KeyT>(c, keys_in, keys_out, vals_in, vals_out, m, c->rp.rank_bits, false, nullptr, 0, c->rp.key_bits == c->rp.rank_bits);
    scan_and_apply(c, m, RecHead<KeyT>{keys_out, vals_out}, RecScatter<KeyT>{keys_out, vals_out, m, recpos, post}, d_u);
    return keys_out;
}
const void *pdl_query_dictionary(pdl_ctx *c, const uint8_t *res, const uint64_t *off, const uint64_t *kmer_off, uint32_t n, uint64_t m,
                                 uint64_t n_res, void *keys_a, void *keys_b, uint32_t *vals_a, uint32_t *vals_b, uint32_t *recpos, uint2 *post,
                                 uint64_t *d_u) {
    if (c->key64) return query_dictionary<uint64_t>(c, res, off, kmer_off, n, m, n_res, (uint64_t *) keys_a, (uint64_t *) keys_b, vals_a, vals_b, recpos, post, d_u);
    return query_dictionary<uint32_t>(c, res, off, kmer_off, n, m, n_res, (uint32_t *) keys_a, (uint32_t *) keys_b, vals_a, vals_b, recpos, post, d_u);
}

template <class KeyT>
static void append_sorted_stream(pdl_ctx *c, uint32_t n, uint64_t m, uint64_t n_res, uint32_t n_base, uint64_t m_base) {
    auto &q = c->qb;
    KeyT *k_in = q.keys_a.as<KeyT>(), *k_out = q.keys_b.as<KeyT>();
    uint32_t *v_in = q.vals_a.as<uint32_t>(), *v_out = q.vals_b.as<uint32_t>();
    ev_begin(c, EV_RANK);
    rank_new_genes<KeyT>(c, q.res.as<uint8_t>(), q.off.as<uint64_t>(), q.koff.as<uint64_t>(), n, m, n_res, k_in, v_in);
    ev_end(c, EV_RANK);
    ev_begin(c, EV_SORT1);
    pdl_sort_pairs<KeyT>(c, k_in, k_out, v_in, v_out, m, c->rp.rank_bits, false, nullptr, 0, c->rp.key_bits == c->rp.rank_bits);
    ev_end(c, EV_SORT1);
    const uint32_t sorted_bits = c->rp.key_bits == c->rp.rank_bits ? 64u : std::min<uint32_t>(64u, 8u * ((c->rp.rank_bits + 7) / 8));
    const KeyT mask = sorted_bits >= 8 * sizeof(KeyT) ? (KeyT) ~(KeyT) 0 : (KeyT) (((KeyT) 1 << (sorted_bits & (8 * sizeof(KeyT) - 1))) - 1);
    ev_begin(c, EV_MERGE);
    pdl_merge_streams<KeyT>(c->stream, c->keys_b.as<KeyT>(), c->vals_b.as<uint32_t>(), (uint32_t) m_base, k_out, v_out, (uint32_t) m, n_base, mask,
                            c->scan_tmp.as<uint32_t>(), c->keys_a.as<KeyT>(), c->vals_a.as<uint32_t>());
    ev_end(c, EV_MERGE);
    std::swap(c->keys_a.p, c->keys_b.p); std::swap(c->keys_a.bytes, c->keys_b.bytes);
    std::swap(c->vals_a.p, c->vals_b.p); std::swap(c->vals_a.bytes, c->vals_b.bytes);
}

void pdl_run_append(pdl_ctx *c, const uint8_t *residues, const uint64_t *offsets, const uint32_t *genome_ids, uint32_t n, uint32_t n_new_genomes,
                    pdl_append_info *info) {
    hipStream_t st = c->stream;
    auto &q = c->qb;
    const uint32_t N0 = c->N, G0 = c->G, k = c->rp.k;
    const uint64_t M0 = c->M, U0 = c->U;
    if ((uint64_t) N0 + n >= 0x7fffffffull) PDL_FAIL(PDL_ERR_UNSUPPORTED, "%llu genes in the union exceed the 31-bit gene ids", (unsigned long long) N0 + n);
    const uint64_t r0 = offsets[0], Rq = offsets[n] - r0;
    if (c->R + Rq >= 0xfffffff0ull) PDL_FAIL(PDL_ERR_UNSUPPORTED, "more than 2^32 residues in the union need 64-bit stream positions");
    std::vector<uint64_t> h_off(n + 1), h_koff(n + 1);
    std::vector<uint32_t> h_kseq(n), h_glen(n);
    uint64_t m = 0;
    for (uint32_t g = 0; g < n; g++) {
        const uint64_t len = offsets[g + 1] - offsets[g];
        h_glen[g] = (uint32_t) len;
        h_off[g] = offsets[g] - r0;
        h_koff[g] = m;
        h_kseq[g] = len >= k ? (uint32_t) (len - k + 1) : 0u;
        m += h_kseq[g];
    }
    h_off[n] = Rq; h_koff[n] = m;
    if (M0 + m >= 0xfffff000ull) PDL_FAIL(PDL_ERR_UNSUPPORTED, "%llu k-mers in the union need 64-bit stream positions", (unsigned long long) (M0 + m));
    for (hipEvent_t &e : c->app_ev) if (!e) PDL_HIP(hipEventCreate(&e));

    PDL_HIP(hipEventRecord(c->app_ev[0], st));
    q.ctl.alloc(16 * sizeof(uint64_t));
    unsigned long long *d_bad = q.ctl.as<unsigned long long>();
    PDL_HIP(hipMemsetAsync(d_bad, 0, sizeof(uint64_t), st));
    q.res.alloc(Rq + 16); q.off.alloc((n + 1) * 8ull); q.koff.alloc((n + 1) * 8ull); q.kseq.alloc(n * 4ull);
    if (Rq) PDL_HIP(hipMemcpyAsync(q.res.p, residues + r0, Rq, hipMemcpyHostToDevice, st));
    PDL_HIP(hipMemcpyAsync(q.off.p, h_off.data(), (n + 1) * 8ull, hipMemcpyHostToDevice, st));
    PDL_HIP(hipMemcpyAsync(q.koff.p, h_koff.data(), (n + 1) * 8ull, hipMemcpyHostToDevice, st));
    PDL_HIP(hipMemcpyAsync(q.kseq.p, h_kseq.data(), n * 4ull, hipMemcpyHostToDevice, st));
    pdl_check_alphabet(c, q.res.as<uint8_t>(), Rq, d_bad);
    PDL_HIP(hipEventRecord(c->app_ev[1], st));
    {
        PinRead rd(c);
        const uint64_t *pb = rd.add<uint64_t>(d_bad, 1);
        rd.sync();
        if (pb[0]) pdl_fail_absent_byte(pb[0], "appended");
    }

    c->preprocessed = false; c->scored = false; c->tasks_ready = false; c->reshard_pending = false;
    c->mirror_valid = false; c->edges_valid = false;
    const uint32_t N1 = N0 + n, G1 = G0 + n_new_genomes;
    const uint64_t M1 = M0 + m;
    const size_t kb = c->key64 ? 8 : 4;
    c->kseq_len.grow_keep((size_t) N1 * sizeof(uint32_t), st);
    c->gene_len.grow_keep((size_t) N1 * sizeof(uint32_t), st);
    c->cost.alloc((size_t) N1 * sizeof(uint64_t));
    const bool ids_on_device = c->d_gen && (c->d_gen == c->in_gen.p || c->d_gen == c->ing_gen.p);
    const bool ids_owned = c->d_gen && c->d_gen == c->own_gen.p;
    if (ids_owned) c->own_gen.grow_keep((size_t) N1 * sizeof(uint32_t), st); else c->own_gen.alloc((size_t) N1 * sizeof(uint32_t));
    const uint32_t *old_gen = c->d_gen;
    pdl_extend_layout(c, genome_ids, n);
    c->M = M1; c->R += Rq;
    c->d_gen = c->own_gen.as<uint32_t>(); c->d_res = nullptr; c->d_off = nullptr;
    const size_t ctl_words = PDL_CTL_GCOST + 2 * (size_t) G1;
    c->scalars.alloc(ctl_words * sizeof(uint64_t));
    if (m) {
        c->keys_a.alloc(M1 * kb); c->vals_a.alloc(M1 * sizeof(uint32_t));
        q.keys_a.alloc(m * kb); q.keys_b.alloc(m * kb); q.vals_a.alloc(m * 4); q.vals_b.alloc(m * 4);
        c->scan_tmp.alloc(pdl_merge_split_words(M1) * sizeof(uint32_t));
    }

    PDL_HIP(hipEventRecord(c->app_ev[2], st));
    uint64_t *d_scal = c->scalars.as<uint64_t>();
    hipLaunchKernelGGL(k_zero_u64, dim3((uint32_t) std::min<size_t>((ctl_words + 255) / 256, 1024)), dim3(256), 0, st, d_scal, ctl_words);
    hipLaunchKernelGGL(k_zero_u64, dim3((uint32_t) std::min<size_t>(((size_t) N1 + 255) / 256, 1024)), dim3(256), 0, st, c->cost.as<uint64_t>(), (size_t) N1);
    PDL_HIP(hipGetLastError());
    PDL_HIP(hipMemcpyAsync(c->kseq_len.as<uint32_t>() + N0, q.kseq.p, n * 4ull, hipMemcpyDeviceToDevice, st));
    PDL_HIP(hipMemcpyAsync(c->gene_len.as<uint32_t>() + N0, h_glen.data(), n * 4ull, hipMemcpyHostToDevice, st));
    if (ids_owned) {
        PDL_HIP(hipMemcpyAsync(c->own_gen.as<uint32_t>() + N0, c->h_genome_of.data() + N0, n * 4ull, hipMemcpyHostToDevice, st));
    } else if (ids_on_device) {
        PDL_HIP(hipMemcpyAsync(c->own_gen.p, old_gen, (size_t) N0 * 4, hipMemcpyDeviceToDevice, st));
        PDL_HIP(hipMemcpyAsync(c->own_gen.as<uint32_t>() + N0, c->h_genome_of.data() + N0, n * 4ull, hipMemcpyHostToDevice, st));
    } else {
        PDL_HIP(hipMemcpyAsync(c->own_gen.p, c->h_genome_of.data(), (size_t) N1 * 4, hipMemcpyHostToDevice, st));
    }
    c->ev[EV_RANK].used = c->ev[EV_SORT1].used = c->ev[EV_MERGE].used = false;
    if (m) {
        if (c->key64) append_sorted_stream<uint64_t>(c, n, m, Rq, N0, M0);
        else append_sorted_stream<uint32_t>(c, n, m, Rq, N0, M0);
    }
    if (c->key64) stage_dedup<uint64_t>(c, M1); else stage_dedup<uint32_t>(c, M1);
    ev_end(c, EV_DICT);
    pdl_prepare_tasks(c);
    stage_ranges_and_costs(c, M1, 1, false);
    PDL_HIP(hipEventRecord(c->app_ev[3], st));
// ... 462 lines not shown
```

pandelos_amd/csrc/pdl_scan.h:

```cpp
#pragma once

#include "pdl_common.h"

#include <type_traits>

template <class T, class = void> struct scan_two_phase : std::false_type {};
template <class T> struct scan_two_phase<T, std::void_t<typename T::Loaded>> : std::true_type {};

constexpr int SCAN_THREADS = 256;
constexpr int SCAN_ITEMS = 8;
constexpr int SCAN_TILE = SCAN_THREADS * SCAN_ITEMS;

__device__ __forceinline__ uint32_t wave_inclusive_scan_u32(uint32_t v) {
    const int lane = threadIdx.x & (PDL_WAVE - 1);
#pragma unroll
    for (int d = 1; d < PDL_WAVE; d <<= 1) {
        uint32_t o = __shfl_up(v, d, PDL_WAVE);
        if (lane >= d) v += o;
    }
    return v;
}

__device__ __forceinline__ uint32_t block_exclusive_scan_u32(uint32_t v, uint32_t *s_wave , uint32_t &total) {
    const int lane = threadIdx.x & (PDL_WAVE - 1);
    const int wave = threadIdx.x / PDL_WAVE;
    const int nw = blockDim.x / PDL_WAVE;
    uint32_t inc = wave_inclusive_scan_u32(v);
    if (lane == PDL_WAVE - 1) s_wave[wave] = inc;
    pdl_sync();
    if (threadIdx.x == 0) {
        uint32_t run = 0;
        for (int w = 0; w < nw; w++) { uint32_t t = s_wave[w]; s_wave[w] = run; run += t; }
        s_wave[16] = run;
    }
    pdl_sync();
    uint32_t res = inc - v + s_wave[wave];
    total = s_wave[16];
    pdl_sync();
    return res;
}

__device__ __forceinline__ uint64_t scan_count(uint64_t n, const uint64_t *d_n) {
    if (!d_n) return n;
    const uint64_t v = *d_n;
    return v < n ? v : n;
}

template <class FlagF>
__global__ __launch_bounds__(SCAN_THREADS) void k_scan_tile_sums(FlagF flag, uint64_t n_bound, const uint64_t *d_n, uint32_t *tile_sums) {
    __shared__ uint32_t s_wave[17];
    const uint64_t n = scan_count(n_bound, d_n);
    if ((uint64_t) blockIdx.x * SCAN_TILE >= n) {
        if (threadIdx.x == 0) tile_sums[blockIdx.x] = 0;
        return;
    }
    const uint64_t base = (uint64_t) blockIdx.x * SCAN_TILE;
    uint32_t sum = 0;
#pragma unroll
    for (int j = 0; j < SCAN_ITEMS; j++) {
        const uint64_t i = base + (uint64_t) j * SCAN_THREADS + threadIdx.x;
        const uint32_t f = flag(i < n ? i : n - 1);
        sum += i < n ? f : 0u;
    }
    uint32_t total;
    (void) block_exclusive_scan_u32(sum, s_wave, total);
    if (threadIdx.x == 0) tile_sums[blockIdx.x] = total;
}

static __global__ __launch_bounds__(1024) void k_scan_tile_scan(uint32_t *tile_sums, uint32_t n_tiles, uint64_t *d_total, uint64_t *d_total2) {
    __shared__ uint32_t s_wave[17];
    __shared__ uint32_t s_carry;
    if (threadIdx.x == 0) s_carry = 0;
    pdl_sync();
    for (uint32_t base = 0; base < n_tiles; base += 1024) {
        uint32_t i = base + threadIdx.x;
        uint32_t v = i < n_tiles ? tile_sums[i] : 0;
        uint32_t total;
        uint32_t ex = block_exclusive_scan_u32(v, s_wave, total);
        uint32_t carry = s_carry;
        if (i < n_tiles) tile_sums[i] = ex + carry;
        pdl_sync();
        if (threadIdx.x == 0) s_carry = carry + total;
        pdl_sync();
    }
    if (threadIdx.x == 0) {
        *d_total = s_carry;
        if (d_total2) {
            reinterpret_cast<uint32_t *>(d_total2)[0] = s_carry;
            reinterpret_cast<uint32_t *>(d_total2)[1] = 0u;
        }
    }
}

constexpr uint32_t SCAN_INLINE_TILES = 1024;
template <class FlagF, class ApplyF, bool INLINE_PREFIX>
__global__ __launch_bounds__(SCAN_THREADS) void k_scan_apply(FlagF flag, ApplyF apply, uint64_t n_bound, const uint64_t *d_n, const uint32_t *tile_sums,
                                                            uint64_t *d_total, uint64_t *d_total2) {
    __shared__ uint32_t s_flags[SCAN_TILE];
    __shared__ uint32_t s_pref[SCAN_TILE];
    __shared__ uint32_t s_wave[17];
    const uint64_t n = scan_count(n_bound, d_n);
    const uint64_t base = (uint64_t) blockIdx.x * SCAN_TILE;
    uint32_t tile_prefix = 0;
    if constexpr (INLINE_PREFIX) {
        const uint32_t upto = blockIdx.x == 0 ? gridDim.x : blockIdx.x;
        uint32_t part = 0;
        for (uint32_t i = threadIdx.x; i < upto; i += SCAN_THREADS) part += tile_sums[i];
        uint32_t all;
        (void) block_exclusive_scan_u32(part, s_wave, all);
        if (blockIdx.x == 0) {
            if (threadIdx.x == 0) {
                *d_total = all;
                if (d_total2) { reinterpret_cast<uint32_t *>(d_total2)[0] = all; reinterpret_cast<uint32_t *>(d_total2)[1] = 0u; }
            }
        } else {
            tile_prefix = all;
        }
    } else {
        tile_prefix = tile_sums[blockIdx.x];
    }
    if (base >= n) return;
#pragma unroll
    for (int j = 0; j < SCAN_ITEMS; j++) {
        const uint32_t li = j * SCAN_THREADS + threadIdx.x;
        const uint64_t i = base + li;
        const uint32_t f = flag(i < n ? i : n - 1);
        s_flags[li] = i < n ? f : 0u;
    }
    pdl_sync();
    uint32_t f[SCAN_ITEMS];
    uint32_t sum = 0;
#pragma unroll
    for (int j = 0; j < SCAN_ITEMS; j++) { f[j] = s_flags[threadIdx.x * SCAN_ITEMS + j]; sum += f[j]; }
    uint32_t total;
    uint32_t prefix = block_exclusive_scan_u32(sum, s_wave, total) + tile_prefix;
#pragma unroll
    for (int j = 0; j < SCAN_ITEMS; j++) { s_pref[threadIdx.x * SCAN_ITEMS + j] = prefix; prefix += f[j]; }
    pdl_sync();
    if constexpr (scan_two_phase<ApplyF>::value) {
        typename ApplyF::Loaded v[SCAN_ITEMS];
#pragma unroll
        for (int j = 0; j < SCAN_ITEMS; j++) {
            const uint32_t li = j * SCAN_THREADS + threadIdx.x;
            const uint64_t i = base + li;
            v[j] = apply.load(i < n ? i : n - 1, s_flags[li]);
        }
#pragma unroll
        for (int j = 0; j < SCAN_ITEMS; j++) {
            const uint32_t li = j * SCAN_THREADS + threadIdx.x;
            const uint64_t i = base + li;
            if (i < n) apply.store(i, s_flags[li], s_pref[li], v[j]);
        }
    } else {
#pragma unroll
        for (int j = 0; j < SCAN_ITEMS; j++) {
            uint32_t li = j * SCAN_THREADS + threadIdx.x;
            uint64_t i = base + li;
            if (i < n) apply(i, s_flags[li], s_pref[li]);
        }
    }
}

constexpr uint32_t LB_CHUNK = PDL_WAVE;
constexpr uint32_t LB_MAX_POLLS = 1u << 22;
constexpr uint32_t LB_CTR_WORDS = 16;
struct LookbackArgs {
    unsigned long long *tile_agg, *chunk_agg, *chunk_incl;
    uint32_t *ctr;
    uint32_t epoch;
};
__device__ __forceinline__ unsigned long long lb_pack(uint32_t epoch, uint32_t value) { return (unsigned long long) epoch << 32 | value; }
__device__ __forceinline__ void lb_publish(unsigned long long *p, uint32_t epoch, uint32_t value) {
    __hip_atomic_store(p, lb_pack(epoch, value), __ATOMIC_RELAXED, __HIP_MEMORY_SCOPE_AGENT);
}
__device__ __forceinline__ uint32_t lb_wait(const unsigned long long *p, uint32_t epoch, uint32_t *err) {
    for (uint32_t polls = 0;; polls++) {
        const unsigned long long w = __hip_atomic_load(p, __ATOMIC_RELAXED, __HIP_MEMORY_SCOPE_AGENT);
        if ((uint32_t) (w >> 32) == epoch) return (uint32_t) w;
        if (polls >= LB_MAX_POLLS) { atomicAdd(err, 1u); return 0u; }
        __builtin_amdgcn_s_sleep(1);
    }
}
__device__ __forceinline__ uint32_t lb_wave_sum(uint32_t v) {
#pragma unroll
    for (int d = PDL_WAVE / 2; d > 0; d >>= 1) v += __shfl_xor(v, d, PDL_WAVE);
    return v;
}
__device__ __forceinline__ uint32_t lb_tile_prefix(const LookbackArgs &lb, uint32_t tile, uint32_t tiles, uint32_t total) {
    const uint32_t lane = threadIdx.x & (PDL_WAVE - 1);
    const uint32_t c = tile / LB_CHUNK, i = tile % LB_CHUNK;
    uint32_t *err = lb.ctr + 2;
    if (lane == 0) lb_publish(&lb.tile_agg[tile], lb.epoch, total);
// ... 156 lines not shown
```

pandelos_amd/csrc/pdl_sort.h:

```cpp
#pragma once

#include "pdl_common.h"

template <class KeyT, class ValT = uint32_t>
void pdl_sort_pairs(pdl_ctx *c, KeyT *&keys_in, KeyT *&keys_out, ValT *&vals_in, ValT *&vals_out,
                    uint64_t n, uint32_t end_bit, bool iota_values = false,
                    const uint64_t *d_n = nullptr,
                    uint32_t begin_bit = 0,
                    bool keys_below_end_bit = false);

constexpr uint32_t PDL_RADIX_TILE = 4096, PDL_RADIX_BINS = 256;
void pdl_radix_offsets(pdl_ctx *c, const uint32_t *counts, uint32_t *offs, uint32_t n_tiles, uint64_t *d_total);

extern template void pdl_sort_pairs<uint32_t, uint32_t>(pdl_ctx *, uint32_t *&, uint32_t *&, uint32_t *&, uint32_t *&, uint64_t, uint32_t, bool, const uint64_t *, uint32_t, bool);
extern template void pdl_sort_pairs<uint64_t, uint32_t>(pdl_ctx *, uint64_t *&, uint64_t *&, uint32_t *&, uint32_t *&, uint64_t, uint32_t, bool, const uint64_t *, uint32_t, bool);
extern template void pdl_sort_pairs<uint32_t, unsigned long long>(pdl_ctx *, uint32_t *&, uint32_t *&, unsigned long long *&, unsigned long long *&, uint64_t, uint32_t, bool, const uint64_t *, uint32_t, bool);
```

pandelos_amd/csrc/pdl_sort.hip:

```cpp
#include "pdl_sort.h"
#include "pdl_scan.h"

constexpr int RS_THREADS = 256;
constexpr int RS_WAVES = RS_THREADS / PDL_WAVE;
constexpr int RS_ROUNDS = 16;
constexpr int RS_TILE = RS_THREADS * RS_ROUNDS;
constexpr int RS_WAVE_SPAN = PDL_WAVE * RS_ROUNDS;
constexpr int RS_BINS = 256;
static_assert(RS_THREADS == RS_BINS, "one thread per digit in the tile-level scans");

template <class KeyT>
__device__ __forceinline__ uint32_t rs_digit(KeyT k, uint32_t shift) { return (uint32_t) (k >> shift) & 0xffu; }

template <class KeyT>
__global__ __launch_bounds__(RS_THREADS) void k_rs_hist(const KeyT *__restrict__ keys, uint64_t n_bound, const uint64_t *d_n, uint32_t shift,
                                                        uint32_t n_tiles, uint32_t *__restrict__ counts) {
    __shared__ uint32_t s_h[RS_BINS];
    const uint64_t n = scan_count(n_bound, d_n);
    const uint64_t base = (uint64_t) blockIdx.x * RS_TILE;
    if (base >= n) {
        counts[(size_t) threadIdx.x * n_tiles + blockIdx.x] = 0;
        return;
    }
    s_h[threadIdx.x] = 0;
    pdl_sync();
    KeyT key[RS_ROUNDS];
#pragma unroll
    for (int j = 0; j < RS_ROUNDS; j++) {
        const uint64_t i = base + (uint64_t) j * RS_THREADS + threadIdx.x;
        key[j] = keys[i < n ? i : n - 1];
    }
#pragma unroll
    for (int j = 0; j < RS_ROUNDS; j++) {
        const uint64_t i = base + (uint64_t) j * RS_THREADS + threadIdx.x;
        if (i < n) atomicAdd(&s_h[rs_digit(key[j], shift)], 1u);
    }
    pdl_sync();
    counts[(size_t) threadIdx.x * n_tiles + blockIdx.x] = s_h[threadIdx.x];
}

struct RsCountFlag {
    const uint32_t *counts;
    __device__ uint32_t operator()(uint64_t i) const { return counts[i]; }
};
struct RsOffsApply {
    uint32_t *offs;
    __device__ void operator()(uint64_t i, uint32_t, uint32_t prefix) const { offs[i] = prefix; }
};

template <class KeyT, class ValT>
__global__ __launch_bounds__(RS_THREADS) void k_rs_scatter(const KeyT *__restrict__ keys_in, const ValT *vals_in,
                                                           KeyT *__restrict__ keys_out, ValT *__restrict__ vals_out, uint64_t n_bound,
                                                           const uint64_t *d_n, uint32_t shift, uint32_t n_tiles, const uint32_t *__restrict__ offs,
                                                           uint32_t nbits) {
    const uint64_t n = scan_count(n_bound, d_n);
    if ((uint64_t) blockIdx.x * (RS_THREADS * RS_ROUNDS) >= n) return;
    __shared__ KeyT s_key[RS_TILE];
    __shared__ ValT s_val[RS_TILE];
    __shared__ uint32_t s_cnt[RS_WAVES][RS_BINS];
    __shared__ uint32_t s_tile_off[RS_BINS];
    __shared__ uint32_t s_goff[RS_BINS];
    __shared__ uint32_t s_wsum[17];

    const uint32_t tid = threadIdx.x, lane = tid & (PDL_WAVE - 1), wave = tid / PDL_WAVE;
    const uint64_t tile_base = (uint64_t) blockIdx.x * RS_TILE;
    const uint64_t wave_base = tile_base + (uint64_t) wave * RS_WAVE_SPAN;
    for (int w = 0; w < RS_WAVES; w++) s_cnt[w][tid] = 0;
    s_goff[tid] = offs[(size_t) tid * n_tiles + blockIdx.x];
    pdl_sync();

    KeyT key[RS_ROUNDS];
    ValT val[RS_ROUNDS];
    uint16_t rank[RS_ROUNDS];
#pragma unroll
    for (int j = 0; j < RS_ROUNDS; j++) {
        const uint64_t i = wave_base + (uint64_t) j * PDL_WAVE + lane;
        key[j] = keys_in[i < n ? i : n - 1];
    }
    if (vals_in) {
#pragma unroll
        for (int j = 0; j < RS_ROUNDS; j++) {
            const uint64_t i = wave_base + (uint64_t) j * PDL_WAVE + lane;
            val[j] = vals_in[i < n ? i : n - 1];
        }
    } else {
#pragma unroll
        for (int j = 0; j < RS_ROUNDS; j++) val[j] = (ValT) (wave_base + (uint64_t) j * PDL_WAVE + lane);
    }
#pragma unroll
    for (int j = 0; j < RS_ROUNDS; j++) {
        const uint64_t i = wave_base + (uint64_t) j * PDL_WAVE + lane;
        const bool valid = i < n;
        const uint32_t d = rs_digit(key[j], shift);
        unsigned long long same = __ballot(valid);
#pragma unroll
        for (int b = 0; b < 8; b++) {
            if ((uint32_t) b >= nbits) break;
            const unsigned long long m = __ballot((d >> b) & 1u);
            same &= ((d >> b) & 1u) ? m : ~m;
        }
        const uint32_t before = s_cnt[wave][d];
        const uint32_t below_me = __builtin_amdgcn_mbcnt_hi((uint32_t) (same >> 32), __builtin_amdgcn_mbcnt_lo((uint32_t) same, 0u));
        rank[j] = (uint16_t) (before + below_me);
        if (valid && below_me == 0) s_cnt[wave][d] = before + (uint32_t) __popcll(same);
    }
    pdl_sync();
    uint32_t tot = 0;
    uint32_t wcnt[RS_WAVES];
#pragma unroll
    for (int w = 0; w < RS_WAVES; w++) { wcnt[w] = s_cnt[w][tid]; tot += wcnt[w]; }
    uint32_t tile_total;
    const uint32_t ex = block_exclusive_scan_u32(tot, s_wsum, tile_total);
    s_tile_off[tid] = ex;
    uint32_t run = ex;
#pragma unroll
    for (int w = 0; w < RS_WAVES; w++) { s_cnt[w][tid] = run; run += wcnt[w]; }
    pdl_sync();
#pragma unroll
    for (int j = 0; j < RS_ROUNDS; j++) {
        const uint64_t i = wave_base + (uint64_t) j * PDL_WAVE + lane;
        if (i < n) {
            const uint32_t lp = s_cnt[wave][rs_digit(key[j], shift)] + rank[j];
            s_key[lp] = key[j];
            s_val[lp] = val[j];
        }
    }
    pdl_sync();
#pragma unroll
    for (int j = 0; j < RS_ROUNDS; j++) {
        const uint32_t e = j * RS_THREADS + tid;
        if (e < tile_total) {
            const KeyT k = s_key[e];
            const uint32_t d = rs_digit(k, shift);
            const uint64_t dst = (uint64_t) s_goff[d] + (e - s_tile_off[d]);
            keys_out[dst] = k;
            vals_out[dst] = s_val[e];
        }
    }
}

template <class KeyT, class ValT>
void pdl_sort_pairs(pdl_ctx *c, KeyT *&keys_in, KeyT *&keys_out, ValT *&vals_in, ValT *&vals_out,
                    uint64_t n, uint32_t end_bit, bool iota_values, const uint64_t *d_n, uint32_t begin_bit, bool keys_below_end_bit) {
    if (n == 0) return;
    if (end_bit == 0) end_bit = 1;
    if (end_bit > sizeof(KeyT) * 8) end_bit = sizeof(KeyT) * 8;
    if (n >= 0xfffff000ull) PDL_FAIL(PDL_ERR_UNSUPPORTED, "sort of %llu pairs needs 64-bit positions", (unsigned long long) n);
    const uint32_t n_tiles = (uint32_t) ((n + RS_TILE - 1) / RS_TILE);
    const size_t table = (size_t) RS_BINS * n_tiles;
    c->sort_tmp.alloc(2 * table * sizeof(uint32_t));
    uint32_t *counts = c->sort_tmp.as<uint32_t>(), *offs = counts + table;
    uint64_t *d_total = c->scalars.as<uint64_t>() + PDL_CTL_SCAN_TOTAL;
    const uint32_t passes = (end_bit + 7) / 8;
    for (uint32_t p = begin_bit / 8; p < passes; p++) {
        const uint32_t shift = p * 8;
        hipLaunchKernelGGL((k_rs_hist<KeyT>), dim3(n_tiles), dim3(RS_THREADS), 0, c->stream, keys_in, n, d_n, shift, n_tiles, counts);
        scan_and_apply(c, table, RsCountFlag{counts}, RsOffsApply{offs}, d_total);
        hipLaunchKernelGGL((k_rs_scatter<KeyT, ValT>), dim3(n_tiles), dim3(RS_THREADS), 0, c->stream, keys_in,
                           (p == begin_bit / 8 && iota_values) ? (const ValT *) nullptr : vals_in, keys_out, vals_out, n, d_n, shift, n_tiles, offs,
                           keys_below_end_bit ? std::min<uint32_t>(8, end_bit - shift) : 8u);
        PDL_HIP(hipGetLastError());
        std::swap(keys_in, keys_out);
        std::swap(vals_in, vals_out);
    }
    std::swap(keys_in, keys_out);
    std::swap(vals_in, vals_out);
}

void pdl_radix_offsets(pdl_ctx *c, const uint32_t *counts, uint32_t *offs, uint32_t n_tiles, uint64_t *d_total) {
    static_assert(PDL_RADIX_TILE == RS_TILE && PDL_RADIX_BINS == RS_BINS, "the caller's kernels use the tile shape of the sort");
    scan_and_apply(c, (size_t) RS_BINS * n_tiles, RsCountFlag{counts}, RsOffsApply{offs}, d_total);
}

template void pdl_sort_pairs<uint32_t, uint32_t>(pdl_ctx *, uint32_t *&, uint32_t *&, uint32_t *&, uint32_t *&, uint64_t, uint32_t, bool, const uint64_t *, uint32_t, bool);
template void pdl_sort_pairs<uint64_t, uint32_t>(pdl_ctx *, uint64_t *&, uint64_t *&, uint32_t *&, uint32_t *&, uint64_t, uint32_t, bool, const uint64_t *, uint32_t, bool);
template void pdl_sort_pairs<uint32_t, unsigned long long>(pdl_ctx *, uint32_t *&, uint32_t *&, unsigned long long *&, unsigned long long *&, uint64_t, uint32_t, bool, const uint64_t *, uint32_t, bool);
```

Measured before the change: 1436 billion.

## Fuse first radix histogram into rank kernel and use per-digit row scans

The rank kernel now builds the first radix pass's per-tile digit histogram, so the sort skips its first histogram launch. The global scan over the whole count table is replaced by a per-digit row scan kernel that writes digit totals. Each scatter kernel then adds the cross-digit prefix itself through a dual block scan. This cuts full passes over the count table and decoupled-lookback scan launches in the dictionary and gene sorts. In exchange it adds shared atomics in the rank kernel, a bigger scatter scan, and a size-based fallback to the old scan path.

```diff
diff --git a/pandelos_amd/csrc/pdl_api.hip b/pandelos_amd/csrc/pdl_api.hip
--- a/pandelos_amd/csrc/pdl_api.hip
+++ b/pandelos_amd/csrc/pdl_api.hip
@@ -610,6 +610,10 @@
     else if (n == "staging_cap") c->opt_staging_cap = value > 0 ? (uint64_t) value : 0;
     else if (n == "aside_test_reload") c->opt_aside_test_reload = value != 0;
     else if (n == "onepass_scan") c->opt_onepass_scan = value != 0;
+    else if (n == "radix_row_tiles") {
+        if (value < 0 || value > 0xffffffffll) { c->err = "radix_row_tiles: a tile count"; return PDL_ERR_ARGUMENT; }
+        c->opt_radix_row_tiles = (uint32_t) value;
+    }
     else if (n == "low_memory") c->opt_low_memory = value != 0;
     else if (n == "query_batch_bytes") {
         if (value <= 0) { c->err = "query_batch_bytes: a positive byte count"; return PDL_ERR_ARGUMENT; }
diff --git a/pandelos_amd/csrc/pdl_common.h b/pandelos_amd/csrc/pdl_common.h
--- a/pandelos_amd/csrc/pdl_common.h
+++ b/pandelos_amd/csrc/pdl_common.h
@@ -235,6 +235,7 @@
     uint32_t lb_epoch = 0;
     bool opt_low_memory = false;
     bool reshard_pending = false;
+    uint32_t opt_radix_row_tiles = 8192;
     bool opt_onepass_scan = false;
     DevBuf scratch;
     DevBuf scalars;
diff --git a/pandelos_amd/csrc/pdl_dict.hip b/pandelos_amd/csrc/pdl_dict.hip
--- a/pandelos_amd/csrc/pdl_dict.hip
+++ b/pandelos_amd/csrc/pdl_dict.hip
@@ -102,6 +102,8 @@
 constexpr int RANK_THREADS = 256;
 constexpr int RANK_ITEMS = 4;
 constexpr int RANK_TILE = RANK_THREADS * RANK_ITEMS;
+constexpr int RANK_TRIPS = (int) PDL_RADIX_TILE / RANK_TILE;
+static_assert(RANK_TRIPS * RANK_TILE == (int) PDL_RADIX_TILE && RANK_THREADS == (int) PDL_RADIX_BINS, "a K-rank workgroup fills one column of the sort's histogram");
 
 __device__ __forceinline__ uint32_t upper_bound_u64(const uint64_t *a, uint32_t lo, uint32_t hi, uint64_t v) {
     while (lo < hi) {
@@ -129,11 +131,14 @@
     __shared__ uint8_t s_rv[256];
     __shared__ uint32_t s_lo, s_hi;
     __shared__ uint64_t s_koff[RANK_SPAN + 1], s_off[RANK_SPAN];
-    __shared__ uint32_t s_bins[MODE == 1 ? DIST_BINS : 1];
+    __shared__ uint32_t s_bins[MODE == 1 ? DIST_BINS : MODE == 2 ? PDL_RADIX_BINS : 1];
     for (int i = threadIdx.x; i < 256; i += RANK_THREADS) s_rv[i] = rp.rank_values[i];
-    if constexpr (MODE == 1) for (uint32_t i = threadIdx.x; i < DIST_BINS; i += RANK_THREADS) s_bins[i] = 0;
+    if constexpr (MODE != 0) for (uint32_t i = threadIdx.x; i < (MODE == 1 ? DIST_BINS : PDL_RADIX_BINS); i += RANK_THREADS) s_bins[i] = 0;
     const uint64_t tiles = (m + RANK_TILE - 1) / RANK_TILE;
-  for (uint64_t tile = blockIdx.x; tile < tiles; tile += gridDim.x) {
+    constexpr uint32_t trips = MODE == 2 ? RANK_TRIPS : 1;
+    const uint64_t tile_first = MODE == 1 ? blockIdx.x : (uint64_t) blockIdx.x * trips;
+    const uint64_t tile_end = MODE == 1 ? tiles : min(tile_first + trips, tiles), tile_step = MODE == 1 ? gridDim.x : 1;
+  for (uint64_t tile = tile_first; tile < tile_end; tile += tile_step) {
     pdl_sync();
     const uint64_t q0 = tile * RANK_TILE;
     const uint64_t q_last = min(q0 + RANK_TILE, m) - 1;
@@ -198,6 +203,7 @@
         const uint64_t q = q0 + (uint64_t) j * RANK_THREADS + threadIdx.x;
         if (q < m) {
             if constexpr (MODE == 1) atomicAdd(&s_bins[(uint32_t) (r[j] >> bin_shift)], 1u);
+            else if constexpr (MODE == 2) atomicAdd(&s_bins[(uint32_t) r[j] & (PDL_RADIX_BINS - 1)], 1u);
             keys[q] = r[j]; vals[q] = sq[j];
         }
     }
@@ -205,6 +211,9 @@
     if constexpr (MODE == 1) {
         pdl_sync();
         for (uint32_t i = threadIdx.x; i < DIST_BINS; i += RANK_THREADS) { const uint32_t v = s_bins[i]; if (v) atomicAdd(&bins[i], v); }
+    } else if constexpr (MODE == 2) {
+        pdl_sync();
+        bins[(size_t) threadIdx.x * gridDim.x + blockIdx.x] = s_bins[threadIdx.x];
     }
 }
 
@@ -723,22 +732,26 @@
 }
 
 __global__ __launch_bounds__(GW_THREADS) void k_range_scatter(GroupTileArgs a, uint32_t n_tiles4, const uint32_t *__restrict__ offs,
-                                                              uint32_t *__restrict__ keys_out, unsigned long long *__restrict__ vals_out) {
+                                                              uint32_t *__restrict__ keys_out, unsigned long long *__restrict__ vals_out,
+                                                              uint64_t *__restrict__ d_total) {
     const uint32_t n = (uint32_t) scan_count(a.n_bound, a.d_n);
-    if ((uint64_t) blockIdx.x * PDL_RADIX_TILE >= n) return;
+    if ((uint64_t) blockIdx.x * PDL_RADIX_TILE >= n) {
+        if (blockIdx.x == 0 && threadIdx.x == 0) *d_total = 0;
+        return;
+    }
     __shared__ uint32_t s_key[PDL_RADIX_TILE];
     __shared__ unsigned long long s_val[PDL_RADIX_TILE];
     __shared__ uint16_t s_cnt[GW_WAVES][PDL_RADIX_BINS];
     __shared__ uint32_t s_tile_off[PDL_RADIX_BINS];
     __shared__ uint32_t s_goff[PDL_RADIX_BINS];
-    __shared__ uint32_t s_wsum[17];
+    __shared__ uint32_t s_wsum[34];
     __shared__ unsigned long long s_own;
     const uint32_t tid = threadIdx.x, lane = tid & (PDL_WAVE - 1), wave = tid / PDL_WAVE;
     const uint32_t tiles = (n + GW_TILE - 1) / GW_TILE;
     const uint32_t tile = blockIdx.x * GW_WAVES + wave, t0 = tile * GW_TILE, t1 = min(t0 + (uint32_t) GW_TILE, n);
     const bool active = tile < tiles;
     for (int w = 0; w < GW_WAVES; w++) s_cnt[w][tid] = 0;
-    s_goff[tid] = offs[(size_t) tid * n_tiles4 + blockIdx.x];
+    const uint32_t run_off = offs[(size_t) tid * n_tiles4 + blockIdx.x], digit_total = offs[(size_t) PDL_RADIX_BINS * n_tiles4 + tid];
     if (tid == 0) s_own = 0;
     pdl_sync();
 
@@ -835,8 +848,12 @@
     uint32_t wcnt[GW_WAVES];
 #pragma unroll
     for (int w = 0; w < GW_WAVES; w++) { wcnt[w] = s_cnt[w][tid]; tot += wcnt[w]; }
-    uint32_t tile_total;
-    const uint32_t ex = block_exclusive_scan_u32(tot, s_wsum, tile_total);
+    uint32_t tile_total, n_ranges;
+    uint32_t ex = tot, below = digit_total;
+    asm volatile("" : "+v"(below));
+    block_exclusive_scan2_u32(ex, below, s_wsum, tile_total, n_ranges);
+    s_goff[tid] = below + run_off;
+    if (blockIdx.x == 0 && tid == 0) *d_total = n_ranges;
     s_tile_off[tid] = ex;
     uint32_t run = ex;
 #pragma unroll
@@ -1030,9 +1047,10 @@
 }
 
 template <class KeyT>
-static void stage_rank(pdl_ctx *c, uint32_t *d_bins = nullptr, uint32_t bin_shift = 0) {
+static bool stage_rank(pdl_ctx *c, uint32_t *d_bins = nullptr, uint32_t bin_shift = 0) {
     hipStream_t st = c->stream;
     const uint64_t M = c->M;
+    bool first_counts = false;
     c->keys_a.alloc(M * sizeof(KeyT)); c->keys_b.alloc(M * sizeof(KeyT));
     c->vals_a.alloc(M * sizeof(uint32_t)); c->vals_b.alloc(M * sizeof(uint32_t));
     if (c->rp.hash_fallback) {
@@ -1046,10 +1064,15 @@
         const uint64_t tiles = (M + RANK_TILE - 1) / RANK_TILE;
         if (d_bins) hipLaunchKernelGGL((k_rank<KeyT, 1>), dim3((uint32_t) std::min<uint64_t>(tiles, 2048)), dim3(RANK_THREADS), 0, st, c->d_res, c->d_off,
                                        c->kmer_off.as<uint64_t>(), c->N, M, c->R, c->rp, c->keys_a.as<KeyT>(), c->vals_a.as<uint32_t>(), bin_shift, d_bins);
-        else hipLaunchKernelGGL((k_rank<KeyT, 0>), dim3((uint32_t) tiles), dim3(RANK_THREADS), 0, st, c->d_res, c->d_off,
-                                c->kmer_off.as<uint64_t>(), c->N, M, c->R, c->rp, c->keys_a.as<KeyT>(), c->vals_a.as<uint32_t>(), 0u, (uint32_t *) nullptr);
+        else {
+            const PdlRadixTables t = pdl_radix_tables(c, M);
+            hipLaunchKernelGGL((k_rank<KeyT, 2>), dim3(t.n_tiles), dim3(RANK_THREADS), 0, st, c->d_res, c->d_off,
+                               c->kmer_off.as<uint64_t>(), c->N, M, c->R, c->rp, c->keys_a.as<KeyT>(), c->vals_a.as<uint32_t>(), 0u, t.counts);
+            first_counts = true;
+        }
     }
     PDL_HIP(hipGetLastError());
+    return first_counts;
 }
 
 template <class KeyT>
@@ -1065,9 +1088,10 @@
 }
 
 template <class KeyT>
-static void stage_sort_and_dedup(pdl_ctx *c, KeyT *keys_in, KeyT *keys_out, uint32_t *vals_in, uint32_t *vals_out, uint64_t m) {
+static void stage_sort_and_dedup(pdl_ctx *c, KeyT *keys_in, KeyT *keys_out, uint32_t *vals_in, uint32_t *vals_out, uint64_t m,
+                                 bool first_counts_ready = false) {
     ev_begin(c, EV_SORT1);
-    pdl_sort_pairs<KeyT>(c, keys_in, keys_out, vals_in, vals_out, m, c->rp.rank_bits, false, nullptr, 0, c->rp.key_bits == c->rp.rank_bits);
+    pdl_sort_pairs<KeyT>(c, keys_in, keys_out, vals_in, vals_out, m, c->rp.rank_bits, false, nullptr, 0, c->rp.key_bits == c->rp.rank_bits, first_counts_ready);
     ev_end(c, EV_SORT1);
     if ((void *) keys_out != c->keys_b.p) { std::swap(c->keys_a.p, c->keys_b.p); std::swap(c->keys_a.bytes, c->keys_b.bytes); }
     if ((void *) vals_out != c->vals_b.p) { std::swap(c->vals_a.p, c->vals_b.p); std::swap(c->vals_a.bytes, c->vals_b.bytes); }
@@ -1162,15 +1186,14 @@
         const uint64_t *d_us = d_scal + PDL_CTL_RANGES;
         const bool fused = mode == 1 && packed;
         if (fused) {
-            const uint32_t n_tiles4 = (uint32_t) ((bound + PDL_RADIX_TILE - 1) / PDL_RADIX_TILE);
-            const size_t table = (size_t) PDL_RADIX_BINS * n_tiles4, tiles = (bound + GW_TILE - 1) / GW_TILE;
-            c->sort_tmp.alloc((2 * table + 3 * tiles + 1) * sizeof(uint32_t));
-            uint32_t *counts = c->sort_tmp.as<uint32_t>(), *offs = counts + table;
-            ga.tile_sums = offs + table; ga.th_first = ga.tile_sums + tiles; ga.th_last = ga.th_first + tiles; ga.chunk_sums = nullptr;
+            const size_t tiles = (bound + GW_TILE - 1) / GW_TILE;
+            const PdlRadixTables rt = pdl_radix_tables(c, bound, 3 * tiles + 1);
+            const uint32_t n_tiles4 = rt.n_tiles;
+            ga.tile_sums = rt.extra(); ga.th_first = ga.tile_sums + tiles; ga.th_last = ga.th_first + tiles; ga.chunk_sums = nullptr;
             const uint32_t grid4 = std::max<uint32_t>(1, std::min<uint32_t>(n_tiles4, (uint32_t) c->cus * 8));
-            hipLaunchKernelGGL(k_range_count_hist, dim3(grid4), dim3(GW_THREADS), 0, st, ga, n_tiles4, counts);
-            pdl_radix_offsets(c, counts, offs, n_tiles4, d_scal + PDL_CTL_RANGES);
-            hipLaunchKernelGGL(k_range_scatter, dim3(n_tiles4), dim3(GW_THREADS), 0, st, ga, n_tiles4, offs, k2b, pay_b);
+            hipLaunchKernelGGL(k_range_count_hist, dim3(grid4), dim3(GW_THREADS), 0, st, ga, n_tiles4, rt.counts);
+            pdl_radix_offsets(c, rt);
+            hipLaunchKernelGGL(k_range_scatter, dim3(n_tiles4), dim3(GW_THREADS), 0, st, ga, n_tiles4, rt.offs, k2b, pay_b, d_scal + PDL_CTL_RANGES);
             PDL_HIP(hipGetLastError());
         } else {
         {
@@ -1204,7 +1227,9 @@
         if (packed) {
             if (fused) {
                 std::swap(k2a, k2b); std::swap(pay_a, pay_b);
+                const void *tables = c->sort_tmp.p;
                 pdl_sort_pairs<uint32_t, unsigned long long>(c, k2a, k2b, pay_a, pay_b, n_sort, seq_bits, false, d_sort_n, 8, true);
+                if (c->sort_tmp.p != tables) PDL_FAIL(PDL_ERR_STATE, "gene sort: the radix tables moved behind the fused first pass");
             } else
             pdl_sort_pairs<uint32_t, unsigned long long>(c, k2a, k2b, pay_a, pay_b, n_sort, seq_bits, false, d_sort_n, 0, true);
             ev_end(c, EV_SORT2);
@@ -1303,11 +1328,11 @@
 static void dictionary_pipeline(pdl_ctx *c, bool only_complexity) {
     const uint64_t M = c->M;
     ev_begin(c, EV_RANK);
-    stage_rank<KeyT>(c);
+    const bool first_counts = stage_rank<KeyT>(c);
     ev_end(c, EV_RANK);
     KeyT *keys_in = c->keys_a.as<KeyT>(), *keys_out = c->keys_b.as<KeyT>();
     uint32_t *vals_in = c->vals_a.as<uint32_t>(), *vals_out = c->vals_b.as<uint32_t>();
-    stage_sort_and_dedup<KeyT>(c, keys_in, keys_out, vals_in, vals_out, M);
+    stage_sort_and_dedup<KeyT>(c, keys_in, keys_out, vals_in, vals_out, M, first_counts);
     ev_end(c, EV_DICT);
     if (c->layout_deferred) pdl_finish_layout(c);
     if (!only_complexity) pdl_prepare_tasks(c);
diff --git a/pandelos_amd/csrc/pdl_scan.h b/pandelos_amd/csrc/pdl_scan.h
--- a/pandelos_amd/csrc/pdl_scan.h
+++ b/pandelos_amd/csrc/pdl_scan.h
@@ -38,6 +38,33 @@
     total = s_wave[16];
     pdl_sync();
     return res;
+}
+
+__device__ __forceinline__ void block_exclusive_scan2_u32(uint32_t &a, uint32_t &b, uint32_t *s_wave , uint32_t &total_a, uint32_t &total_b) {
+    const int lane = threadIdx.x & (PDL_WAVE - 1);
+    const int wave = threadIdx.x / PDL_WAVE;
+    const int nw = blockDim.x / PDL_WAVE;
+    uint32_t ia = a, ib = b;
+#pragma unroll
+    for (int d = 1; d < PDL_WAVE; d <<= 1) {
+        const uint32_t oa = __shfl_up(ia, d, PDL_WAVE), ob = __shfl_up(ib, d, PDL_WAVE);
+        if (lane >= d) { ia += oa; ib += ob; }
+    }
+    if (lane == PDL_WAVE - 1) { s_wave[wave] = ia; s_wave[17 + wave] = ib; }
+    pdl_sync();
+    if (threadIdx.x == 0) {
+        uint32_t ra = 0, rb = 0;
+        for (int w = 0; w < nw; w++) {
+            const uint32_t ta = s_wave[w], tb = s_wave[17 + w];
+            s_wave[w] = ra; s_wave[17 + w] = rb;
+            ra += ta; rb += tb;
+        }
+        s_wave[16] = ra; s_wave[33] = rb;
+    }
+    pdl_sync();
+    a = ia - a + s_wave[wave]; b = ib - b + s_wave[17 + wave];
+    total_a = s_wave[16]; total_b = s_wave[33];
+    pdl_sync();
 }
 
 __device__ __forceinline__ uint64_t scan_count(uint64_t n, const uint64_t *d_n) {
diff --git a/pandelos_amd/csrc/pdl_sort.h b/pandelos_amd/csrc/pdl_sort.h
--- a/pandelos_amd/csrc/pdl_sort.h
+++ b/pandelos_amd/csrc/pdl_sort.h
@@ -1,17 +1,26 @@
 #pragma once
 
 #include "pdl_common.h"
+
+constexpr uint32_t PDL_RADIX_TILE = 4096, PDL_RADIX_BINS = 256;
+struct PdlRadixTables {
+    uint32_t n_tiles;
+    uint32_t *counts, *offs;
+    uint32_t *digit_total() const { return offs + (size_t) PDL_RADIX_BINS * n_tiles; }
+    uint32_t *extra() const { return digit_total() + PDL_RADIX_BINS; }
+};
+PdlRadixTables pdl_radix_tables(pdl_ctx *c, uint64_t n, size_t extra_words = 0);
 
 template <class KeyT, class ValT = uint32_t>
 void pdl_sort_pairs(pdl_ctx *c, KeyT *&keys_in, KeyT *&keys_out, ValT *&vals_in, ValT *&vals_out,
                     uint64_t n, uint32_t end_bit, bool iota_values = false,
                     const uint64_t *d_n = nullptr,
                     uint32_t begin_bit = 0,
-                    bool keys_below_end_bit = false);
+                    bool keys_below_end_bit = false,
+                    bool first_counts_ready = false);
 
-constexpr uint32_t PDL_RADIX_TILE = 4096, PDL_RADIX_BINS = 256;
-void pdl_radix_offsets(pdl_ctx *c, const uint32_t *counts, uint32_t *offs, uint32_t n_tiles, uint64_t *d_total);
+void pdl_radix_offsets(pdl_ctx *c, const PdlRadixTables &t);
 
-extern template void pdl_sort_pairs<uint32_t, uint32_t>(pdl_ctx *, uint32_t *&, uint32_t *&, uint32_t *&, uint32_t *&, uint64_t, uint32_t, bool, const uint64_t *, uint32_t, bool);
-extern template void pdl_sort_pairs<uint64_t, uint32_t>(pdl_ctx *, uint64_t *&, uint64_t *&, uint32_t *&, uint32_t *&, uint64_t, uint32_t, bool, const uint64_t *, uint32_t, bool);
-extern template void pdl_sort_pairs<uint32_t, unsigned long long>(pdl_ctx *, uint32_t *&, uint32_t *&, unsigned long long *&, unsigned long long *&, uint64_t, uint32_t, bool, const uint64_t *, uint32_t, bool);
+extern template void pdl_sort_pairs<uint32_t, uint32_t>(pdl_ctx *, uint32_t *&, uint32_t *&, uint32_t *&, uint32_t *&, uint64_t, uint32_t, bool, const uint64_t *, uint32_t, bool, bool);
+extern template void pdl_sort_pairs<uint64_t, uint32_t>(pdl_ctx *, uint64_t *&, uint64_t *&, uint32_t *&, uint32_t *&, uint64_t, uint32_t, bool, const uint64_t *, uint32_t, bool, bool);
+extern template void pdl_sort_pairs<uint32_t, unsigned long long>(pdl_ctx *, uint32_t *&, uint32_t *&, unsigned long long *&, unsigned long long *&, uint64_t, uint32_t, bool, const uint64_t *, uint32_t, bool, bool);
diff --git a/pandelos_amd/csrc/pdl_sort.hip b/pandelos_amd/csrc/pdl_sort.hip
--- a/pandelos_amd/csrc/pdl_sort.hip
+++ b/pandelos_amd/csrc/pdl_sort.hip
@@ -39,14 +39,24 @@
     counts[(size_t) threadIdx.x * n_tiles + blockIdx.x] = s_h[threadIdx.x];
 }
 
-struct RsCountFlag {
-    const uint32_t *counts;
-    __device__ uint32_t operator()(uint64_t i) const { return counts[i]; }
-};
-struct RsOffsApply {
-    uint32_t *offs;
-    __device__ void operator()(uint64_t i, uint32_t, uint32_t prefix) const { offs[i] = prefix; }
-};
+constexpr int RO_THREADS = 1024;
+__global__ __launch_bounds__(RO_THREADS) void k_rs_offsets(const uint32_t *__restrict__ counts, uint32_t *__restrict__ offs, uint32_t n_tiles) {
+    __shared__ uint32_t s_wave[17];
+    const uint32_t *row = counts + (size_t) blockIdx.x * n_tiles;
+    uint32_t *out = offs + (size_t) blockIdx.x * n_tiles;
+    uint32_t carry = 0;
+    uint32_t v = threadIdx.x < n_tiles ? row[threadIdx.x] : 0u;
+    for (uint32_t base = 0; base < n_tiles; base += RO_THREADS) {
+        const uint32_t i = base + threadIdx.x;
+        const uint32_t v_next = i + RO_THREADS < n_tiles ? row[i + RO_THREADS] : 0u;
+        uint32_t total;
+        const uint32_t ex = block_exclusive_scan_u32(v, s_wave, total);
+        if (i < n_tiles) out[i] = carry + ex;
+        carry += total;
+        v = v_next;
+    }
+    if (threadIdx.x == 0) offs[(size_t) RS_BINS * n_tiles + blockIdx.x] = carry;
+}
 
 template <class KeyT, class ValT>
 __global__ __launch_bounds__(RS_THREADS) void k_rs_scatter(const KeyT *__restrict__ keys_in, const ValT *vals_in,
@@ -60,13 +70,13 @@
     __shared__ uint32_t s_cnt[RS_WAVES][RS_BINS];
     __shared__ uint32_t s_tile_off[RS_BINS];
     __shared__ uint32_t s_goff[RS_BINS];
-    __shared__ uint32_t s_wsum[17];
+    __shared__ uint32_t s_wsum[34];
 
     const uint32_t tid = threadIdx.x, lane = tid & (PDL_WAVE - 1), wave = tid / PDL_WAVE;
     const uint64_t tile_base = (uint64_t) blockIdx.x * RS_TILE;
     const uint64_t wave_base = tile_base + (uint64_t) wave * RS_WAVE_SPAN;
     for (int w = 0; w < RS_WAVES; w++) s_cnt[w][tid] = 0;
-    s_goff[tid] = offs[(size_t) tid * n_tiles + blockIdx.x];
+    const uint32_t run_off = offs[(size_t) tid * n_tiles + blockIdx.x], digit_total = offs[(size_t) RS_BINS * n_tiles + tid];
     pdl_sync();
 
     KeyT key[RS_ROUNDS];
@@ -109,8 +119,11 @@
     uint32_t wcnt[RS_WAVES];
 #pragma unroll
     for (int w = 0; w < RS_WAVES; w++) { wcnt[w] = s_cnt[w][tid]; tot += wcnt[w]; }
-    uint32_t tile_total;
-    const uint32_t ex = block_exclusive_scan_u32(tot, s_wsum, tile_total);
+    uint32_t tile_total, n_all;
+    uint32_t ex = tot, below = digit_total;
+    asm volatile("" : "+v"(below));
+    block_exclusive_scan2_u32(ex, below, s_wsum, tile_total, n_all);
+    s_goff[tid] = below + run_off;
     s_tile_off[tid] = ex;
     uint32_t run = ex;
 #pragma unroll
@@ -141,23 +154,21 @@
 
 template <class KeyT, class ValT>
 void pdl_sort_pairs(pdl_ctx *c, KeyT *&keys_in, KeyT *&keys_out, ValT *&vals_in, ValT *&vals_out,
-                    uint64_t n, uint32_t end_bit, bool iota_values, const uint64_t *d_n, uint32_t begin_bit, bool keys_below_end_bit) {
+                    uint64_t n, uint32_t end_bit, bool iota_values, const uint64_t *d_n, uint32_t begin_bit, bool keys_below_end_bit,
+                    bool first_counts_ready) {
     if (n == 0) return;
     if (end_bit == 0) end_bit = 1;
     if (end_bit > sizeof(KeyT) * 8) end_bit = sizeof(KeyT) * 8;
-    if (n >= 0xfffff000ull) PDL_FAIL(PDL_ERR_UNSUPPORTED, "sort of %llu pairs needs 64-bit positions", (unsigned long long) n);
-    const uint32_t n_tiles = (uint32_t) ((n + RS_TILE - 1) / RS_TILE);
-    const size_t table = (size_t) RS_BINS * n_tiles;
-    c->sort_tmp.alloc(2 * table * sizeof(uint32_t));
-    uint32_t *counts = c->sort_tmp.as<uint32_t>(), *offs = counts + table;
-    uint64_t *d_total = c->scalars.as<uint64_t>() + PDL_CTL_SCAN_TOTAL;
+    const PdlRadixTables t = pdl_radix_tables(c, n);
+    const uint32_t n_tiles = t.n_tiles;
     const uint32_t passes = (end_bit + 7) / 8;
     for (uint32_t p = begin_bit / 8; p < passes; p++) {
         const uint32_t shift = p * 8;
-        hipLaunchKernelGGL((k_rs_hist<KeyT>), dim3(n_tiles), dim3(RS_THREADS), 0, c->stream, keys_in, n, d_n, shift, n_tiles, counts);
-        scan_and_apply(c, table, RsCountFlag{counts}, RsOffsApply{offs}, d_total);
+        if (!(first_counts_ready && p == begin_bit / 8))
+            hipLaunchKernelGGL((k_rs_hist<KeyT>), dim3(n_tiles), dim3(RS_THREADS), 0, c->stream, keys_in, n, d_n, shift, n_tiles, t.counts);
+        pdl_radix_offsets(c, t);
         hipLaunchKernelGGL((k_rs_scatter<KeyT, ValT>), dim3(n_tiles), dim3(RS_THREADS), 0, c->stream, keys_in,
-                           (p == begin_bit / 8 && iota_values) ? (const ValT *) nullptr : vals_in, keys_out, vals_out, n, d_n, shift, n_tiles, offs,
+                           (p == begin_bit / 8 && iota_values) ? (const ValT *) nullptr : vals_in, keys_out, vals_out, n, d_n, shift, n_tiles, t.offs,
                            keys_below_end_bit ? std::min<uint32_t>(8, end_bit - shift) : 8u);
         PDL_HIP(hipGetLastError());
         std::swap(keys_in, keys_out);
@@ -167,11 +178,40 @@
     std::swap(vals_in, vals_out);
 }
 
-void pdl_radix_offsets(pdl_ctx *c, const uint32_t *counts, uint32_t *offs, uint32_t n_tiles, uint64_t *d_total) {
-    static_assert(PDL_RADIX_TILE == RS_TILE && PDL_RADIX_BINS == RS_BINS, "the caller's kernels use the tile shape of the sort");
-    scan_and_apply(c, (size_t) RS_BINS * n_tiles, RsCountFlag{counts}, RsOffsApply{offs}, d_total);
-}
-
-template void pdl_sort_pairs<uint32_t, uint32_t>(pdl_ctx *, uint32_t *&, uint32_t *&, uint32_t *&, uint32_t *&, uint64_t, uint32_t, bool, const uint64_t *, uint32_t, bool);
-template void pdl_sort_pairs<uint64_t, uint32_t>(pdl_ctx *, uint64_t *&, uint64_t *&, uint32_t *&, uint32_t *&, uint64_t, uint32_t, bool, const uint64_t *, uint32_t, bool);
-template void pdl_sort_pairs<uint32_t, unsigned long long>(pdl_ctx *, uint32_t *&, uint32_t *&, unsigned long long *&, unsigned long long *&, uint64_t, uint32_t, bool, const uint64_t *, uint32_t, bool);
+PdlRadixTables pdl_radix_tables(pdl_ctx *c, uint64_t n, size_t extra_words) {
+    static_assert(PDL_RADIX_TILE == RS_TILE && PDL_RADIX_BINS == RS_BINS, "the callers' kernels use the tile shape of the sort");
+    if (n >= 0xfffff000ull) PDL_FAIL(PDL_ERR_UNSUPPORTED, "sort of %llu pairs needs 64-bit positions", (unsigned long long) n);
+    PdlRadixTables t{};
+    t.n_tiles = (uint32_t) ((n + RS_TILE - 1) / RS_TILE);
+    const size_t table = (size_t) RS_BINS * t.n_tiles;
+    c->sort_tmp.alloc((2 * table + RS_BINS + extra_words) * sizeof(uint32_t));
+    t.counts = c->sort_tmp.as<uint32_t>();
+    t.offs = t.counts + table;
+    return t;
+}
+
+struct RsCountFlag {
+    const uint32_t *counts;
+    __device__ uint32_t operator()(uint64_t i) const { return counts[i]; }
+};
+struct RsOffsApply {
+    uint32_t *offs;
+    __device__ void operator()(uint64_t i, uint32_t, uint32_t prefix) const { offs[i] = prefix; }
+};
+__global__ __launch_bounds__(RS_BINS) void k_rs_total_in_last_digit(const uint64_t *__restrict__ d_total, uint32_t *__restrict__ digit_total) {
+    digit_total[threadIdx.x] = threadIdx.x == RS_BINS - 1 ? (uint32_t) *d_total : 0u;
+}
+
+void pdl_radix_offsets(pdl_ctx *c, const PdlRadixTables &t) {
+    if (t.n_tiles <= c->opt_radix_row_tiles) {
+        hipLaunchKernelGGL(k_rs_offsets, dim3(RS_BINS), dim3(RO_THREADS), 0, c->stream, t.counts, t.offs, t.n_tiles);
+        return;
+    }
+    uint64_t *d_total = c->scalars.as<uint64_t>() + PDL_CTL_SCAN_TOTAL;
+    scan_and_apply(c, (size_t) RS_BINS * t.n_tiles, RsCountFlag{t.counts}, RsOffsApply{t.offs}, d_total);
+    hipLaunchKernelGGL(k_rs_total_in_last_digit, dim3(1), dim3(RS_BINS), 0, c->stream, d_total, t.digit_total());
+}
+
+template void pdl_sort_pairs<uint32_t, uint32_t>(pdl_ctx *, uint32_t *&, uint32_t *&, uint32_t *&, uint32_t *&, uint64_t, uint32_t, bool, const uint64_t *, uint32_t, bool, bool);
+template void pdl_sort_pairs<uint64_t, uint32_t>(pdl_ctx *, uint64_t *&, uint64_t *&, uint32_t *&, uint32_t *&, uint64_t, uint32_t, bool, const uint64_t *, uint32_t, bool, bool);
+template void pdl_sort_pairs<uint32_t, unsigned long long>(pdl_ctx *, uint32_t *&, uint32_t *&, unsigned long long *&, unsigned long long *&, uint64_t, uint32_t, bool, const uint64_t *, uint32_t, bool, bool);
```

Result: faster. 1456 billion, median of 6 (+1.4%).
